# Sorax5/RaytracingEngine

Hardware: AMD Instinct MI355X
Metric: Mrays/sec (primary+shadow) at 1920x1080 (higher is better)
Workload: dtype f64

## Files before the change

### include/rt_capi.h

```cpp
#ifndef RT_CAPI_H
#define RT_CAPI_H

#include <stddef.h>
#include <stdint.h>

#ifdef __cplusplus
extern "C" {
#endif

#define RT_CAPI_VERSION 1

typedef enum rt_status {
    RT_OK = 0,
    RT_ERR_INVALID_ARG = 1,
    RT_ERR_HIP = 2,
    RT_ERR_OOM = 3,
    RT_ERR_UNSUPPORTED = 4,
    RT_ERR_NO_DEVICE = 5,
    RT_ERR_RCCL = 6
} rt_status;

typedef struct rt_material {
    double color[3];
    double shininess;
// ... 197 lines not shown
                            int nframes, const rt_render_opts* opts, int outputs,
                            const struct rt_gbuffer* d_out);
rt_status rt_gbuffer(rt_context* ctx, const rt_scene* scene, const rt_camera* cam,
                     const rt_render_opts* opts, int outputs, const struct rt_gbuffer* h_out);

typedef struct rt_queue rt_queue;
rt_status rt_queue_create(rt_context* ctx, int depth, rt_queue** out);
rt_status rt_queue_destroy(rt_queue* queue);
rt_status rt_queue_submit(rt_queue* queue, const rt_scene* scene, const rt_camera* cam,
                          const rt_render_opts* opts, void* d_hdr64, void* d_hdr32, void* d_ldr,
                          uint64_t* ticket);
rt_status rt_queue_wait(rt_queue* queue, uint64_t ticket);
rt_status rt_queue_synchronize(rt_queue* queue);

rt_status rt_stats_read(rt_context* ctx, rt_stats* out);
rt_status rt_stats_reset(rt_context* ctx);

rt_status rt_trace_rays(rt_context* ctx, const rt_scene* scene, const rt_render_opts* opts,
                        const double* rays, size_t n, double* rgb_out, rt_stats* stats);

rt_status rt_intersect_rays(rt_context* ctx, const rt_scene* scene, const double* rays,
                            size_t n, double* hits_out);

rt_status rt_occluded_rays(rt_context* ctx, const rt_scene* scene, const rt_render_opts* opts,
                           const double* rays, const double* max_dist, size_t n,
                           uint8_t* occluded_out);
rt_status rt_occluded_rays_device(rt_context* ctx, const rt_scene* scene,
                                  const rt_render_opts* opts, const void* d_rays,
                                  const void* d_max_dist, size_t n, void* d_occluded);

rt_status rt_transmittance_rays(rt_context* ctx, const rt_scene* scene, const rt_render_opts* opts,
                                const double* rays, const double* max_dist, size_t n,
                                double* T_out);
rt_status rt_transmittance_rays_device(rt_context* ctx, const rt_scene* scene,
                                       const rt_render_opts* opts, const void* d_rays,
                                       const void* d_max_dist, size_t n, void* d_T);

rt_status rt_light_transmittance(rt_context* ctx, const rt_scene* scene, const rt_render_opts* opts,
                                 const double* points, size_t n, double* T_out);
rt_status rt_light_transmittance_device(rt_context* ctx, const rt_scene* scene,
                                        const rt_render_opts* opts, const void* d_points, size_t n,
                                        void* d_T);

#define RT_DL_RADIANCE 0x1
#define RT_DL_DIFFUSE  0x2
#define RT_DL_SPECULAR 0x4
#define RT_DL_ALL      0x7
struct rt_direct_light_out {
    void* radiance;
    void* diffuse;
    void* specular;
};
rt_status rt_direct_light(rt_context* ctx, const rt_scene* scene, const rt_render_opts* opts,
                          const double* points, const rt_material* materials, size_t n_materials,
                          size_t n, int outputs, const struct rt_direct_light_out* out);
rt_status rt_direct_light_device(rt_context* ctx, const rt_scene* scene,
                                 const rt_render_opts* opts, const void* d_points,
                                 const void* d_materials, size_t n_materials, size_t n,
                                 int outputs, const struct rt_direct_light_out* d_out);

rt_status rt_direct_light_rays(rt_context* ctx, const rt_scene* scene, const rt_render_opts* opts,
                               const double* rays, size_t n, int outputs,
                               const struct rt_direct_light_out* out);
rt_status rt_direct_light_rays_device(rt_context* ctx, const rt_scene* scene,
                                      const rt_render_opts* opts, const void* d_rays, size_t n,
                                      int outputs, const struct rt_direct_light_out* d_out);

#define RT_SC_VALUE    0x01
#define RT_SC_REFRACT  0x02
#define RT_SC_REFLECT  0x04
#define RT_SC_WEIGHTS  0x08
#define RT_SC_FLAGS    0x10
#define RT_SC_ALL      0x1f
struct rt_scatter_out {
    void* value;
    void* refract_rays;
    void* reflect_rays;
    void* weights;
    void* flags;
};
rt_status rt_scatter_rays(rt_context* ctx, const rt_scene* scene, const rt_render_opts* opts,
                          const double* rays, size_t n, int outputs,
                          const struct rt_scatter_out* out);
rt_status rt_scatter_rays_device(rt_context* ctx, const rt_scene* scene,
                                 const rt_render_opts* opts, const void* d_rays, size_t n,
                                 int outputs, const struct rt_scatter_out* d_out);

rt_status rt_camera_rays(rt_context* ctx, const rt_camera* cam, const rt_render_opts* opts,
                         int sample, double* rays_out);
rt_status rt_camera_rays_device(rt_context* ctx, const rt_camera* cam, const rt_render_opts* opts,
                                int sample, void* d_rays);

#define RT_CH_T        0x01
#define RT_CH_PRIM     0x02
#define RT_CH_NORMAL   0x04
#define RT_CH_POINT    0x08
#define RT_CH_MATERIAL 0x10
#define RT_CH_ALL      0x1f
struct rt_closest_out {
    void* t;
    void* prim;
    void* normal;
    void* point;
    void* material;
};
rt_status rt_closest_rays(rt_context* ctx, const rt_scene* scene, const rt_render_opts* opts,
                          const double* rays, size_t n, int outputs,
                          const struct rt_closest_out* out);
rt_status rt_closest_rays_device(rt_context* ctx, const rt_scene* scene,
                                 const rt_render_opts* opts, const void* d_rays, size_t n,
                                 int outputs, const struct rt_closest_out* d_out);

rt_status rt_trace_rays_device(rt_context* ctx, const rt_scene* scene, const rt_render_opts* opts,
                               const void* d_rays, size_t n, void* d_rgb);

rt_status rt_accumulate_samples_device(rt_context* ctx, const rt_scene* scene,
                                       const rt_camera* cam, const rt_render_opts* opts,
                                       int sample_begin, int sample_end, void* d_sum);
rt_status rt_accumulate_samples(rt_context* ctx, const rt_scene* scene, const rt_camera* cam,
                                const rt_render_opts* opts, int sample_begin, int sample_end,
                                double* sum);

rt_status rt_resolve_device(rt_context* ctx, const void* d_sum, size_t n_pixels, int samples,
                            int tonemap, void* d_hdr64, void* d_hdr32, void* d_ldr);
rt_status rt_resolve(rt_context* ctx, const double* sum, size_t n_pixels, int samples, int tonemap,
                     double* hdr64, float* hdr32, uint8_t* ldr);

rt_status rt_tonemap(rt_context* ctx, const double* hdr, size_t n_pixels, int op,
                     uint8_t* ldr_out);

rt_status rt_debug_f64_ops(rt_context* ctx, const double* x, const double* y, size_t n,
                           double* out);

rt_status rt_debug_vec_ops(rt_context* ctx, const double* v, size_t n, double* out);

rt_status rt_debug_assemble_rows(rt_context* ctx, const void* gathered, size_t row_bytes,
                                 uint32_t height, uint32_t block, uint32_t n, uint32_t max_rows,
                                 void* image);

rt_status rt_debug_tile_order(rt_context* ctx, const rt_scene* scene, const rt_camera* cam,
                              uint32_t* order, uint32_t* cost, size_t capacity, uint32_t* tiles,
                              uint32_t* waves, int* state);

rt_status rt_debug_cone_table(rt_context* ctx, uint64_t* with_table, uint64_t* without_table);

rt_status rt_debug_shadow_table(rt_context* ctx, uint64_t* with_table, uint64_t* without_table);

rt_status rt_debug_tile_class(rt_context* ctx, uint64_t* with_words, uint64_t* without_words);

rt_status rt_debug_plane_clear(rt_context* ctx, uint64_t* with_masks, uint64_t* without_masks);

rt_status rt_debug_tile_split(rt_context* ctx, uint64_t* split, uint64_t* single);

#ifdef __cplusplus
}
#endif

#endif
```

### raytracingengine_amd/capi.py

```python
from __future__ import annotations

import ctypes
import os

import numpy as np

from .scene import AREA_LIGHT_DTYPE, SceneData

HERE = os.path.dirname(os.path.abspath(__file__))
LIB_PATH = os.environ.get("RTAMD_LIB", os.path.join(HERE, "librtamd.so"))

(RT_OK, RT_ERR_INVALID_ARG, RT_ERR_HIP, RT_ERR_OOM, RT_ERR_UNSUPPORTED, RT_ERR_NO_DEVICE,
 RT_ERR_RCCL) = range(7)
STATUS_NAMES = {0: "RT_OK", 1: "RT_ERR_INVALID_ARG", 2: "RT_ERR_HIP", 3: "RT_ERR_OOM",
                4: "RT_ERR_UNSUPPORTED", 5: "RT_ERR_NO_DEVICE", 6: "RT_ERR_RCCL"}

TONEMAP_NONE = -1
TONEMAPS = ["simple", "reinhard_simple", "reinhard_extended", "reinhard_extended_luminance",
            "reinhard_jodie", "uncharted2", "aces"]
TONEMAP_ALL = 7
RT_FLAG_COUNT_RAYS = 0x1
RT_FLAG_TIME_KERNEL = 0x2
RT_FLAG_GENERIC_KERNEL = 0x4
RT_FLAG_NO_BVH = 0x8
RT_FLAG_PIPELINE = 0x10
RT_FLAG_NO_TILE_ORDER = 0x20
RT_FLAG_NO_SAMPLE_PARALLEL = 0x40
RT_OUT_HDR64, RT_OUT_HDR32, RT_OUT_LDR = 0x1, 0x2, 0x4
RT_COMM_ID_BYTES = 128
GB_DEPTH = 0x01
GB_DEPTH_NORM = 0x02
GB_NORMAL = 0x04
GB_PRIM = 0x08
GB_ALBEDO = 0x10
GB_ALL = 0x1F
DL_RADIANCE = 0x1
DL_DIFFUSE = 0x2
DL_SPECULAR = 0x4
DL_ALL = 0x7
DL_OUTPUTS = [("radiance", DL_RADIANCE), ("diffuse", DL_DIFFUSE), ("specular", DL_SPECULAR)]
SC_VALUE = 0x01
SC_REFRACT = 0x02
SC_REFLECT = 0x04
SC_WEIGHTS = 0x08
SC_FLAGS = 0x10
SC_ALL = 0x1F
SC_OUTPUTS = [("value", SC_VALUE, np.float64, 3), ("refract_rays", SC_REFRACT, np.float64, 6),
              ("reflect_rays", SC_REFLECT, np.float64, 6), ("weights", SC_WEIGHTS, np.float64, 2),
              ("flags", SC_FLAGS, np.uint8, 0)]
CH_T = 0x01
CH_PRIM = 0x02
CH_NORMAL = 0x04
CH_POINT = 0x08
CH_MATERIAL = 0x10
CH_ALL = 0x1F
CH_OUTPUTS = [("t", CH_T, np.float64, 0), ("prim", CH_PRIM, np.int32, 2),
              ("normal", CH_NORMAL, np.float64, 3), ("point", CH_POINT, np.float64, 3),
              ("material", CH_MATERIAL, np.float64, 7)]
GB_OUTPUTS = [("depth", GB_DEPTH, np.float64, 1), ("depth_norm", GB_DEPTH_NORM, np.float32, 1),
              ("normal", GB_NORMAL, np.float64, 3), ("prim", GB_PRIM, np.int32, 2),
              ("albedo", GB_ALBEDO, np.float32, 3)]

EXPORTED = [
    "rt_last_error", "rt_build_info", "rt_device_count", "rt_render_opts_default", "rt_context_create",
    "rt_context_destroy", "rt_context_set_stream", "rt_context_synchronize", "rt_scene_create",
    "rt_scene_destroy", "rt_scene_set_area_light", "rt_render", "rt_render_device",
    "rt_render_multi", "rt_comm_unique_id", "rt_comm_create", "rt_comm_create_all",
    "rt_comm_create_local", "rt_comm_destroy", "rt_comm_info", "rt_comm_set_root_weight",
    "rt_comm_create_ex", "rt_comm_set_timeout", "rt_render_gather", "rt_render_gather_all",
    "rt_comm_timing", "rt_comm_synchronize", "rt_debug_assemble_rows", "rt_debug_tile_order",
    "rt_stats_read", "rt_stats_reset", "rt_trace_rays", "rt_intersect_rays", "rt_tonemap",
    "rt_debug_f64_ops", "rt_debug_vec_ops", "rt_queue_create", "rt_queue_destroy",
    "rt_queue_submit", "rt_queue_wait", "rt_queue_synchronize", "rt_render_batch",
    "rt_render_gather_batch", "rt_render_gather_all_batch", "rt_gbuffer", "rt_gbuffer_device",
    "rt_debug_cone_table",
    "rt_debug_shadow_table",
    "rt_debug_tile_class",
    "rt_debug_plane_clear",
    "rt_debug_tile_split",
    "rt_occluded_rays", "rt_occluded_rays_device",
    "rt_transmittance_rays", "rt_transmittance_rays_device",
    "rt_light_transmittance", "rt_light_transmittance_device",
    "rt_direct_light", "rt_direct_light_device",
    "rt_direct_light_rays", "rt_direct_light_rays_device",
    "rt_scatter_rays", "rt_scatter_rays_device",
    "rt_camera_rays", "rt_camera_rays_device",
    "rt_closest_rays", "rt_closest_rays_device",
    "rt_trace_rays_device",
    "rt_accumulate_samples", "rt_accumulate_samples_device",
    "rt_resolve", "rt_resolve_device",
]


class RtError(RuntimeError):
    def __init__(self, status: int, msg: str):
        super().__init__(f"{STATUS_NAMES.get(status, status)}: {msg}")
        self.status = status


class SceneDesc(ctypes.Structure):
    _fields_ = [
        ("spheres", ctypes.c_void_p), ("n_spheres", ctypes.c_int32),
        ("planes", ctypes.c_void_p), ("n_planes", ctypes.c_int32),
        ("triangles", ctypes.c_void_p), ("n_triangles", ctypes.c_int32),
        ("lights", ctypes.c_void_p), ("n_lights", ctypes.c_int32),
    ]


class RenderOpts(ctypes.Structure):
    _fields_ = [
        ("max_recursion", ctypes.c_int32), ("tonemap", ctypes.c_int32),
        ("bias", ctypes.c_double), ("seed", ctypes.c_uint64),
        ("row_begin", ctypes.c_uint32), ("row_end", ctypes.c_uint32),
        ("flags", ctypes.c_int32), ("row_block", ctypes.c_uint16), ("row_cycle", ctypes.c_uint16),
    ]


class Stats(ctypes.Structure):
    _fields_ = [
        ("trace_rays", ctypes.c_uint64), ("shadow_rays", ctypes.c_uint64),
        ("kernel_ms", ctypes.c_double), ("launches", ctypes.c_uint64),
    ]


class GBufferPtrs(ctypes.Structure):
    _fields_ = [(name, ctypes.c_void_p) for name, _, _, _ in GB_OUTPUTS]


def gbuffer_layout(outputs: int, width: int, rows: int, frames: int | None = None) -> dict:
    if outputs == 0 or outputs & ~GB_ALL:
        raise ValueError(f"G-buffer outputs {outputs:#x}: no output or an unknown bit")
    lead = () if frames is None else (int(frames),)
    return {name: (lead + (rows, width) + ((k,) if k > 1 else ()), np.dtype(dt))
            for name, bit, dt, k in GB_OUTPUTS if outputs & bit}


class DirectLightPtrs(ctypes.Structure):
    _fields_ = [(name, ctypes.c_void_p) for name, _ in DL_OUTPUTS]


def material_rows(materials, n: int) -> np.ndarray:
    if hasattr(materials, "as_tuple"):
        c, *rest = materials.as_tuple()
        materials = (*c, *rest)
    m = np.ascontiguousarray(materials, np.float64)
    if m.ndim == 1:
        m = m.reshape(1, -1)
    if m.ndim != 2 or m.shape[1] != 7 or m.shape[0] not in (1, n):
        raise ValueError("materials: a Material, seven values, or an [n, 7] array")
    return m


class ScatterPtrs(ctypes.Structure):
    _fields_ = [(name, ctypes.c_void_p) for name, *_ in SC_OUTPUTS]


def _sc_check(outputs: int):
    if outputs == 0 or outputs & ~SC_ALL:
        raise ValueError("outputs: a non-empty combination of SC_* bits")


class ClosestPtrs(ctypes.Structure):
    _fields_ = [(name, ctypes.c_void_p) for name, *_ in CH_OUTPUTS]


def _ch_check(outputs: int):
    if outputs == 0 or outputs & ~CH_ALL:
        raise ValueError("outputs: a non-empty combination of CH_* bits")


def _dl_check(outputs: int):
    if outputs == 0 or outputs & ~DL_ALL:
        raise ValueError("outputs: a non-empty combination of DL_* bits")


class GatherTiming(ctypes.Structure):
    _fields_ = [
        ("render_ms", ctypes.c_double), ("gather_ms", ctypes.c_double),
        ("assemble_ms", ctypes.c_double), ("frames", ctypes.c_uint64),
        ("rows", ctypes.c_uint32), ("max_rows", ctypes.c_uint32),
    ]


_lib = None


def load_library(path: str = LIB_PATH):
    global _lib
    if _lib is not None:
        return _lib
    try:
        import torch
    except ImportError:
        pass
    if not os.path.exists(path):
        raise RuntimeError(
            f"{path} is missing: build it with `python -c 'import __graft_entry__ as g; g.build()'`"
            " (hipcc --offload-arch=gfx950). The renderer has no CPU fallback.")
    L = ctypes.CDLL(path)
    vp, i32 = ctypes.c_void_p, ctypes.c_int
    L.rt_last_error.restype = ctypes.c_char_p
    if hasattr(L, "rt_build_info") or "RTAMD_LIB" not in os.environ:
        L.rt_build_info.restype = ctypes.c_char_p
        L.rt_build_info.argtypes = []
    L.rt_device_count.restype = i32
    L.rt_render_opts_default.argtypes = [vp]
    L.rt_render_opts_default.restype = None
    for name, args in {
        "rt_context_create": [i32, vp],
        "rt_context_destroy": [vp],
        "rt_context_set_stream": [vp, vp],
        "rt_context_synchronize": [vp],
        "rt_scene_create": [vp, vp, vp],
        "rt_scene_destroy": [vp],
        "rt_scene_set_area_light": [vp, vp],
        "rt_render": [vp, vp, vp, vp, vp, vp, vp, vp],
        "rt_render_device": [vp, vp, vp, vp, vp, vp, vp],
        "rt_render_batch": [vp, vp, vp, i32, vp, vp, vp, vp],
        "rt_gbuffer": [vp, vp, vp, vp, i32, vp],
        "rt_gbuffer_device": [vp, vp, vp, i32, vp, i32, vp],
        "rt_render_multi": [vp, vp, i32, vp, vp, vp, vp, vp, vp],
        "rt_stats_read": [vp, vp],
        "rt_stats_reset": [vp],
        "rt_trace_rays": [vp, vp, vp, vp, ctypes.c_size_t, vp, vp],
        "rt_intersect_rays": [vp, vp, vp, ctypes.c_size_t, vp],
        "rt_occluded_rays": [vp, vp, vp, vp, vp, ctypes.c_size_t, vp],
        "rt_occluded_rays_device": [vp, vp, vp, vp, vp, ctypes.c_size_t, vp],
        "rt_transmittance_rays": [vp, vp, vp, vp, vp, ctypes.c_size_t, vp],
        "rt_transmittance_rays_device": [vp, vp, vp, vp, vp, ctypes.c_size_t, vp],
        "rt_light_transmittance": [vp, vp, vp, vp, ctypes.c_size_t, vp],
        "rt_light_transmittance_device": [vp, vp, vp, vp, ctypes.c_size_t, vp],
        "rt_direct_light": [vp, vp, vp, vp, vp, ctypes.c_size_t, ctypes.c_size_t, i32, vp],
        "rt_direct_light_device": [vp, vp, vp, vp, vp, ctypes.c_size_t, ctypes.c_size_t, i32, vp],
        "rt_direct_light_rays": [vp, vp, vp, vp, ctypes.c_size_t, i32, vp],
        "rt_direct_light_rays_device": [vp, vp, vp, vp, ctypes.c_size_t, i32, vp],
        "rt_scatter_rays": [vp, vp, vp, vp, ctypes.c_size_t, i32, vp],
        "rt_scatter_rays_device": [vp, vp, vp, vp, ctypes.c_size_t, i32, vp],
        "rt_camera_rays": [vp, vp, vp, i32, vp],
        "rt_camera_rays_device": [vp, vp, vp, i32, vp],
        "rt_closest_rays": [vp, vp, vp, vp, ctypes.c_size_t, i32, vp],
        "rt_closest_rays_device": [vp, vp, vp, vp, ctypes.c_size_t, i32, vp],
        "rt_trace_rays_device": [vp, vp, vp, vp, ctypes.c_size_t, vp],
        "rt_accumulate_samples": [vp, vp, vp, vp, i32, i32, vp],
        "rt_accumulate_samples_device": [vp, vp, vp, vp, i32, i32, vp],
        "rt_resolve": [vp, vp, ctypes.c_size_t, i32, i32, vp, vp, vp],
        "rt_resolve_device": [vp, vp, ctypes.c_size_t, i32, i32, vp, vp, vp],
        "rt_tonemap": [vp, vp, ctypes.c_size_t, i32, vp],
        "rt_debug_f64_ops": [vp, vp, vp, ctypes.c_size_t, vp],
        "rt_debug_vec_ops": [vp, vp, ctypes.c_size_t, vp],
        "rt_comm_unique_id": [vp],
        "rt_comm_create": [vp, i32, i32, vp, vp],
        "rt_comm_create_ex": [vp, i32, i32, vp, ctypes.c_long, vp],
        "rt_comm_set_timeout": [vp, ctypes.c_long],
        "rt_comm_create_all": [vp, i32, vp],
        "rt_comm_create_local": [vp, i32, vp],
        "rt_comm_destroy": [vp],
        "rt_comm_info": [vp, vp, vp],
        "rt_comm_set_root_weight": [vp, i32],
        "rt_render_gather": [vp, vp, vp, vp, i32, vp, vp, vp],
        "rt_render_gather_all": [vp, vp, i32, vp, vp, i32, vp, vp, vp],
        "rt_render_gather_batch": [vp, vp, vp, i32, vp, i32, vp, vp, vp, vp, vp, vp],
        "rt_render_gather_all_batch": [vp, vp, i32, vp, i32, vp, i32, vp, vp, vp],
        "rt_comm_timing": [vp, vp, i32],
        "rt_comm_synchronize": [vp],
        "rt_queue_create": [vp, i32, vp],
        "rt_queue_destroy": [vp],
        "rt_queue_submit": [vp, vp, vp, vp, vp, vp, vp, vp],
        "rt_queue_wait": [vp, ctypes.c_uint64],
        "rt_queue_synchronize": [vp],
        "rt_debug_tile_order": [vp, vp, vp, vp, vp, ctypes.c_size_t, vp, vp, vp],
        "rt_debug_cone_table": [vp, vp, vp],
        "rt_debug_shadow_table": [vp, vp, vp],
        "rt_debug_tile_class": [vp, vp, vp],
        "rt_debug_plane_clear": [vp, vp, vp],
        "rt_debug_tile_split": [vp, vp, vp],
        "rt_debug_assemble_rows": [vp, vp, ctypes.c_size_t, ctypes.c_uint32, ctypes.c_uint32,
                                   ctypes.c_uint32, ctypes.c_uint32, vp],
    }.items():
        try:
            fn = getattr(L, name)
        except AttributeError:
            if "RTAMD_LIB" in os.environ:
                continue
            raise
        fn.argtypes = args
        fn.restype = i32
    _lib = L
    return L


def build_info() -> dict:
    import json
    info = json.loads(load_library().rt_build_info().decode())
    from . import build
    info["matches_tree"] = info.get("source_sha256") == build.source_digest()
    return info


def _check(status: int):
    if status != RT_OK:
        raise RtError(status, _lib.rt_last_error().decode(errors="replace"))


def rendered_rows(o: RenderOpts, height: int) -> int:
    r1 = min(o.row_end, height) if o.row_end else height
    if r1 <= o.row_begin:
        return 0
    if o.row_cycle <= 1 or o.row_block == 0:
        return r1 - o.row_begin
    stride = o.row_block * o.row_cycle
    return sum(min(o.row_block, r1 - b) for b in range(o.row_begin, r1, stride))


def default_opts(**kw) -> RenderOpts:
    o = RenderOpts()
    load_library().rt_render_opts_default(ctypes.byref(o))
    for k, v in kw.items():
        setattr(o, k, v)
    return o


def device_count() -> int:
    return load_library().rt_device_count()


def progressive_schedule(aa_samples: int) -> list:
    n = max(1, int(aa_samples))
    steps, k = [], 1
    while k < n:
        steps.append(k)
        k *= 2
    return steps + [n]


class Context:

    def __init__(self, device: int = 0):
        L = load_library()
        self._h = ctypes.c_void_p()
        _check(L.rt_context_create(device, ctypes.byref(self._h)))
        self.device = device

    def close(self):
        if self._h:
            _lib.rt_context_destroy(self._h)
            self._h = ctypes.c_void_p()

    def __del__(self):
        try:
            self.close()
        except Exception:
            pass

    def __enter__(self):
        return self

    def __exit__(self, *exc):
        self.close()

    @property
    def handle(self):
        return self._h

    def set_stream(self, stream_ptr: int | None):
        _check(_lib.rt_context_set_stream(self._h, stream_ptr))

    def synchronize(self):
        _check(_lib.rt_context_synchronize(self._h))

    def scene(self, sc: SceneData) -> "DeviceScene":
        return DeviceScene(self, sc)

    def stats(self) -> Stats:
        s = Stats()
        _check(_lib.rt_stats_read(self._h, ctypes.byref(s)))
        return s

    def reset_stats(self):
        _check(_lib.rt_stats_reset(self._h))

    def tonemap(self, hdr: np.ndarray, op: int) -> np.ndarray:
        hdr = np.ascontiguousarray(hdr, np.float64).reshape(-1, 3)
        planes = 7 if op == TONEMAP_ALL else 1
        out = np.empty((planes, hdr.shape[0], 3), np.uint8)
        _check(_lib.rt_tonemap(self._h, hdr.ctypes.data, hdr.shape[0], op, out.ctypes.data))
        return out if planes > 1 else out[0]

    def debug_f64_ops(self, x: np.ndarray, y: np.ndarray) -> np.ndarray:
        x = np.ascontiguousarray(x, np.float64)
        y = np.ascontiguousarray(y, np.float64)
        out = np.empty((x.size, 5), np.float64)
        _check(_lib.rt_debug_f64_ops(self._h, x.ctypes.data, y.ctypes.data, x.size,
                                     out.ctypes.data))
        return out

    def debug_assemble_rows(self, gathered: np.ndarray, height: int, block: int, n: int,
                            max_rows: int) -> np.ndarray:
        g = np.ascontiguousarray(gathered, np.uint8).reshape(n, max_rows, -1)
        out = np.empty((height, g.shape[2]), np.uint8)
        _check(_lib.rt_debug_assemble_rows(self._h, g.ctypes.data, g.shape[2], height, block, n,
                                           max_rows, out.ctypes.data))
        return out

    def debug_cone_table(self) -> tuple[int, int]:
        a, b = ctypes.c_uint64(), ctypes.c_uint64()
        _check(_lib.rt_debug_cone_table(self._h, ctypes.byref(a), ctypes.byref(b)))
        return a.value, b.value

    def debug_shadow_table(self) -> tuple[int, int]:
        a, b = ctypes.c_uint64(), ctypes.c_uint64()
        _check(_lib.rt_debug_shadow_table(self._h, ctypes.byref(a), ctypes.byref(b)))
        return a.value, b.value

    def debug_tile_class(self) -> tuple[int, int]:
        a, b = ctypes.c_uint64(), ctypes.c_uint64()
        _check(_lib.rt_debug_tile_class(self._h, ctypes.byref(a), ctypes.byref(b)))
        return a.value, b.value

    def debug_plane_clear(self) -> tuple[int, int]:
        a, b = ctypes.c_uint64(), ctypes.c_uint64()
        _check(_lib.rt_debug_plane_clear(self._h, ctypes.byref(a), ctypes.byref(b)))
        return a.value, b.value

    def debug_tile_split(self) -> tuple[int, int]:
        a, b = ctypes.c_uint64(), ctypes.c_uint64()
        _check(_lib.rt_debug_tile_split(self._h, ctypes.byref(a), ctypes.byref(b)))
        return a.value, b.value

    def debug_vec_ops(self, v: np.ndarray) -> np.ndarray:
        v = np.ascontiguousarray(v, np.float64).reshape(-1, 3)
        out = np.empty((v.shape[0], 16), np.float64)
        _check(_lib.rt_debug_vec_ops(self._h, v.ctypes.data, v.shape[0], out.ctypes.data))
        return out


class DeviceScene:

    def __init__(self, ctx: Context, sc: SceneData):
        self.ctx = ctx
        self.data = sc
        self._arrays = (sc.sphere_array(), sc.plane_array(), sc.triangle_array(), sc.light_array())
        sp, pl, tr, lt = self._arrays
        desc = SceneDesc(sp.ctypes.data if len(sp) else None, len(sp),
                         pl.ctypes.data if len(pl) else None, len(pl),
                         tr.ctypes.data if len(tr) else None, len(tr),
                         lt.ctypes.data if len(lt) else None, len(lt))
        self._h = ctypes.c_void_p()
        _check(_lib.rt_scene_create(ctx.handle, ctypes.byref(desc), ctypes.byref(self._h)))
        self.camera = sc.camera.to_struct()
        self._area = None
        if sc.area_light is not None:
            self._area = sc.area_light.to_struct()
            _check(_lib.rt_scene_set_area_light(self._h, self._area.ctypes.data))

    def close(self):
        if self._h:
            _lib.rt_scene_destroy(self._h)
            self._h = ctypes.c_void_p()

    def __del__(self):
        try:
            self.close()
        except Exception:
            pass

    def render(self, *, hdr64=True, hdr32=False, tonemap: int = TONEMAP_NONE, opts=None,
               stats=False, **opt_kw):
        cam = self.data.camera
        o = opts if opts is not None else default_opts(tonemap=tonemap, **opt_kw)
        if opts is None:
            o.tonemap = tonemap
        rows = rendered_rows(o, cam.height)
        out = {}
        a64 = np.empty((rows, cam.width, 3), np.float64) if hdr64 else None
        a32 = np.empty((rows, cam.width, 3), np.float32) if hdr32 else None
        ldr = np.empty((rows, cam.width, 3), np.uint8) if tonemap != TONEMAP_NONE else None
        st = Stats()
        _check(_lib.rt_render(self.ctx.handle, self._h, self.camera.ctypes.data, ctypes.byref(o),
                              a64.ctypes.data if a64 is not None else None,
                              a32.ctypes.data if a32 is not None else None,
                              ldr.ctypes.data if ldr is not None else None,
                              ctypes.byref(st) if stats else None))
        if a64 is not None:
            out["hdr64"] = a64
        if a32 is not None:
            out["hdr32"] = a32
        if ldr is not None:
            out["ldr"] = ldr
        if stats:
            out["trace_rays"] = st.trace_rays
            out["shadow_rays"] = st.shadow_rays
        return out

    def render_host(self, h_hdr64: int | None, h_hdr32: int | None, h_ldr: int | None,
                    opts: RenderOpts, stats: bool = False):
        st = Stats()
        _check(_lib.rt_render(self.ctx.handle, self._h, self.camera.ctypes.data, ctypes.byref(opts),
                              h_hdr64, h_hdr32, h_ldr, ctypes.byref(st) if stats else None))
        return st if stats else None

    def trace_rays(self, rays: np.ndarray, stats=False, **opt_kw):
        rays = np.ascontiguousarray(rays, np.float64).reshape(-1, 6)
        out = np.empty((rays.shape[0], 3), np.float64)
        o = default_opts(**opt_kw)
        st = Stats()
        _check(_lib.rt_trace_rays(self.ctx.handle, self._h, ctypes.byref(o), rays.ctypes.data,
                                  rays.shape[0], out.ctypes.data,
                                  ctypes.byref(st) if stats else None))
        return (out, st) if stats else out

    def intersect_rays(self, rays: np.ndarray) -> np.ndarray:
        rays = np.ascontiguousarray(rays, np.float64).reshape(-1, 6)
        out = np.empty((rays.shape[0], 9), np.float64)
        _check(_lib.rt_intersect_rays(self.ctx.handle, self._h, rays.ctypes.data, rays.shape[0],
                                      out.ctypes.data))
        return out

    def occluded(self, rays: np.ndarray, max_dist, no_bvh: bool = False) -> np.ndarray:
        rays = np.ascontiguousarray(rays, np.float64).reshape(-1, 6)
        n = rays.shape[0]
        dist = np.ascontiguousarray(np.broadcast_to(np.asarray(max_dist, np.float64), (n,)))
        out = np.empty(n, np.uint8)
        o = default_opts(flags=RT_FLAG_NO_BVH if no_bvh else 0)
        _check(_lib.rt_occluded_rays(self.ctx.handle, self._h, ctypes.byref(o), rays.ctypes.data,
                                     dist.ctypes.data, n, out.ctypes.data))
        return out.view(np.bool_)

    def occluded_device(self, rays, max_dist, out=None, no_bvh: bool = False):
        import torch
        dev = torch.device(f"cuda:{self.ctx.device}")
        if rays.dtype != torch.float64 or rays.device != dev or not rays.is_contiguous():
            raise ValueError("rays: a contiguous float64 tensor on the context's device")
        n = rays.numel() // 6
        if rays.numel() != 6 * n:
            raise ValueError("rays: n*6 elements")
        if not torch.is_tensor(max_dist):
            max_dist = torch.full((n,), float(max_dist), dtype=torch.float64, device=dev)
            torch.cuda.current_stream(dev).synchronize()
        if (max_dist.dtype != torch.float64 or max_dist.device != dev or max_dist.numel() != n
                or not max_dist.is_contiguous()):
            raise ValueError("max_dist: a scalar or a contiguous float64 [n] tensor on the device")
        if out is None:
            out = torch.empty(n, dtype=torch.uint8, device=dev)
        elif (out.dtype != torch.uint8 or out.device != dev or out.numel() < n
              or not out.is_contiguous()):
            raise ValueError("out: a contiguous uint8 tensor of at least n elements on the device")
        o = default_opts(flags=RT_FLAG_NO_BVH if no_bvh else 0)
        _check(_lib.rt_occluded_rays_device(self.ctx.handle, self._h, ctypes.byref(o),
                                            rays.data_ptr() if n else None,
                                            max_dist.data_ptr() if n else None, n,
                                            out.data_ptr() if n else None))
        return out

    def transmittance(self, rays: np.ndarray, max_dist, bias: float = 1e-3,
                      no_bvh: bool = False) -> np.ndarray:
        rays = np.ascontiguousarray(rays, np.float64).reshape(-1, 6)
        n = rays.shape[0]
        dist = np.ascontiguousarray(np.broadcast_to(np.asarray(max_dist, np.float64), (n,)))
        out = np.empty(n, np.float64)
        o = default_opts(bias=bias, flags=RT_FLAG_NO_BVH if no_bvh else 0)
        _check(_lib.rt_transmittance_rays(self.ctx.handle, self._h, ctypes.byref(o),
                                          rays.ctypes.data, dist.ctypes.data, n, out.ctypes.data))
        return out

    def transmittance_device(self, rays, max_dist, out=None, bias: float = 1e-3,
                             no_bvh: bool = False):
        import torch
        dev = torch.device(f"cuda:{self.ctx.device}")
        if rays.dtype != torch.float64 or rays.device != dev or not rays.is_contiguous():
            raise ValueError("rays: a contiguous float64 tensor on the context's device")
        n = rays.numel() // 6
        if rays.numel() != 6 * n:
            raise ValueError("rays: n*6 elements")
        if not torch.is_tensor(max_dist):
            max_dist = torch.full((n,), float(max_dist), dtype=torch.float64, device=dev)
            torch.cuda.current_stream(dev).synchronize()
        if (max_dist.dtype != torch.float64 or max_dist.device != dev or max_dist.numel() != n
                or not max_dist.is_contiguous()):
            raise ValueError("max_dist: a scalar or a contiguous float64 [n] tensor on the device")
        if out is None:
# ... 631 lines not shown
```

### raytracingengine_amd/csrc/rt_capi.cpp

```cpp
#include "rt_capi.h"

#include <hip/hip_runtime.h>

#include <algorithm>
#include <cmath>
#include <cstdlib>
#include <cstdio>
#include <cstring>
#include <mutex>
#include <new>
#include <string>
#include <utility>
#include <vector>

#include "rt_context.hpp"
#include "rt_internal.hpp"
#include "rt_wavefront.hpp"

#pragma clang fp contract(off)

using namespace rtamd;

namespace rtamd {

// ... 171 lines not shown
                                  static_cast<size_t>(kLtStride) * sc->nl);
    lds = lds_bytes <= ctx->lds_limit;
    return RT_OK;
}

bool uses_wavefront_arena(int path, int flags) {
    if (flags & RT_FLAG_GENERIC_KERNEL) return false;
    const char* wf_chain = std::getenv("RTAMD_WF_CHAIN");
    return path == kPathTree || (path == kPathChain && wf_chain && std::atoi(wf_chain) == 1);
}

rt_status scratch_wait(rt_context* ctx) {
    if (ctx->scratch_used && ctx->scratch_stream != ctx->stream)
        RT_HIP(hipStreamWaitEvent(ctx->stream, ctx->scratch_event, 0));
    return RT_OK;
}

rt_status scratch_done(rt_context* ctx) {
    RT_HIP(hipEventRecord(ctx->scratch_event, ctx->stream));
    ctx->scratch_used = true;
    ctx->scratch_stream = ctx->stream;
    return RT_OK;
}

rt_status fixup_buffers(rt_context* ctx, size_t px, TraceParams& p) {
    if (px >= (size_t(1) << 32)) return fail(RT_ERR_UNSUPPORTED, "fix-up list above 2^32 pixels");
    if (!ctx->fix_ctl.ptr) {
        RT_HIP(ctx->fix_ctl.ensure(2 * sizeof(uint32_t)));
        RT_HIP(hipMemsetAsync(ctx->fix_ctl.ptr, 0, 2 * sizeof(uint32_t), ctx->stream));
    }
    if (ctx->fix_list.bytes < px * sizeof(uint32_t)) {
        if (ctx->scratch_used) RT_HIP(hipEventSynchronize(ctx->scratch_event));
        RT_HIP(ctx->fix_list.ensure(px * sizeof(uint32_t)));
    }
    p.fix_list = static_cast<uint32_t*>(ctx->fix_list.ptr);
    p.fix_ctl = static_cast<uint32_t*>(ctx->fix_ctl.ptr) + ctx->fix_parity;
    p.fix_next = static_cast<uint32_t*>(ctx->fix_ctl.ptr) + (1 - ctx->fix_parity);
    return RT_OK;
}

rt_status check_batch(const rt_camera* cams, int nframes) {
    if (!cams || nframes < 1) return fail(RT_ERR_INVALID_ARG, "frame batch: no cameras");
    for (int f = 0; f < nframes; ++f) {
        rt_status st = validate_camera(cams + f);
        if (st != RT_OK) return st;
        if (cams[f].width != cams[0].width || cams[f].height != cams[0].height ||
            cams[f].aa_samples != cams[0].aa_samples ||
            std::memcmp(&cams[f].focal, &cams[0].focal, sizeof(double)) != 0)
            return fail(RT_ERR_INVALID_ARG, "frame batch: every camera must have the first's "
                                            "width, height, focal and aa_samples");
    }
    return RT_OK;
}

rt_status enqueue_render(rt_context* ctx, const rt_scene* sc, const rt_camera* cam,
                         const rt_render_opts* opts, double* d64, float* d32, uint8_t* dldr) {
    return enqueue_frames(ctx, sc, cam, 1, opts, d64, d32, dldr);
}

rt_status enqueue_frames(rt_context* ctx, const rt_scene* sc, const rt_camera* cams, int nframes,
                         const rt_render_opts* opts, double* d64, float* d32, uint8_t* dldr,
                         uint32_t frame_rows) {
    TraceParams p;
    int path;
    bool lds;
    size_t lds_bytes;
    uint32_t rows;
    rt_status st = nframes == 1 ? RT_OK : check_batch(cams, nframes);
    if (st != RT_OK) return st;
    st = build_params(ctx, sc, cams, opts, p, path, lds, lds_bytes, rows);
    if (st != RT_OK) return st;
    p.out64 = d64;
    p.out32 = d32;
    p.ldr = dldr;
    const int flags = opts ? opts->flags : 0;
    if (!dldr) p.tonemap = RT_TONEMAP_NONE;
    if (dldr && p.tonemap == RT_TONEMAP_NONE) p.ldr = nullptr;
    const bool packet_path = path == kPathDirect && !(flags & RT_FLAG_GENERIC_KERNEL) &&
                             p.ns <= packet_max_spheres() &&
                             packet_lds_bytes(p.ns, p.np, p.nl) <= ctx->lds_limit;
    if (frame_rows && frame_rows < rows)
        return fail(RT_ERR_INVALID_ARG, "frame batch: frame stride below the rendered rows");
    const size_t frame_px = static_cast<size_t>(frame_rows ? frame_rows : rows) * p.width;
    if (nframes > 1 && (!packet_path || nframes > kPkMaxBatch)) {
        const int step = packet_path ? kPkMaxBatch : 1;
        for (int f0 = 0; f0 < nframes; f0 += step) {
            const size_t off = 3 * frame_px * static_cast<size_t>(f0);
            st = enqueue_frames(ctx, sc, cams + f0, std::min(step, nframes - f0), opts,
                                d64 ? d64 + off : nullptr, d32 ? d32 + off : nullptr,
                                dldr ? dldr + off : nullptr, frame_rows);
            if (st != RT_OK) return st;
        }
        return RT_OK;
    }
    bool scratch = (flags & RT_FLAG_COUNT_RAYS) || uses_wavefront_arena(path, flags);

    std::pair<hipEvent_t, hipEvent_t> ev{nullptr, nullptr};
    if (flags & RT_FLAG_TIME_KERNEL) {
        if (ctx->pending.size() >= 1024) {
            st = harvest_events(ctx, false);
            if (st != RT_OK) return st;
        }
        if (!ctx->free_events.empty()) {
            ev = ctx->free_events.back();
            ctx->free_events.pop_back();
        } else {
            RT_HIP(hipEventCreate(&ev.first));
            RT_HIP(hipEventCreate(&ev.second));
        }
        RT_HIP(hipEventRecord(ev.first, ctx->stream));
    }
    const bool packet = packet_path;
    rt_scene::PkImage::TileOrder* rec = nullptr;
    int batch_ring = -1;
    PkSplit pk_split{0u, 0u, 0u};
    if (packet && nframes > 1) {
        p.nframes = static_cast<uint32_t>(nframes);
        p.frame_px = frame_px;
        st = packet_batch_images(ctx, sc, cams, nframes, p, flags, &rec, &batch_ring, &pk_split);
        if (st != RT_OK) return st;
    } else if (packet) {
        st = packet_image(ctx, sc, p, flags, &rec);
        if (st != RT_OK) return st;
    }
    if (packet) {
        for (int f = 0; f < nframes; ++f)
            ++((nframes > 1 ? p.fr_tab[f] : p.cone_tab) ? ctx->cone_tab_frames
                                                         : ctx->cone_notab_frames);
        for (int f = 0; f < nframes; ++f)
            ++((nframes > 1 ? p.fr_stab[f] : p.shadow_tab) ? ctx->shadow_tab_frames
                                                            : ctx->shadow_notab_frames);
        for (int f = 0; f < nframes; ++f)
            ++((nframes > 1 ? p.fr_ctab[f] : p.class_tab) ? ctx->tile_class_frames
                                                          : ctx->tile_noclass_frames);
        for (int f = 0; f < nframes; ++f)
            ++(((nframes > 1 ? p.fr_ctab[f] : p.class_tab) && p.plane_masks)
                   ? ctx->plane_mask_frames
                   : ctx->plane_nomask_frames);
    }
    const bool fixup = packet && packet_uses_fixup(p, false, sc->max_specular > 0.0);
    if (fixup) {
        st = fixup_buffers(ctx, nframes > 1 ? static_cast<size_t>(nframes) * frame_px
                                             : static_cast<size_t>(rows) * p.width, p);
        if (st != RT_OK) return st;
        scratch = true;
    }
    if (scratch) {
        st = scratch_wait(ctx);
        if (st != RT_OK) return st;
    }
    if (!fixup || p.tile_order) pk_split.tiles = 0;
    if (packet && fixup)
        (pk_split.tiles ? ctx->tile_split_frames : ctx->tile_nosplit_frames) += nframes;
    const bool lean_generic = p.nt == 0 && p.al_samples == 0;
    static const bool box_sph = [] {
        const char* e = std::getenv("RTAMD_BOX_SPH");
        return !(e && std::atoi(e) == 0);
    }();
    const bool box = path == kPathChain && p.nt == 0 && p.al_samples == 0 &&
                     (p.ns == 0 ? p.np > 0 : (box_sph && p.ns <= kBoxMaxSpheres)) &&
                     !(flags & RT_FLAG_GENERIC_KERNEL);
    const bool spar = !(flags & RT_FLAG_NO_SAMPLE_PARALLEL);
    auto launch = [&](const TraceParams& q, bool count) {
        if (box)
            return launch_box_chain(q, count, !(flags & RT_FLAG_NO_SAMPLE_PARALLEL), ctx->stream);
        return packet ? launch_packet_direct(q, count, sc->max_specular > 0.0, ctx->stream,
                                             count ? nullptr : &pk_split)
                      : (lean_generic ? lean::launch_trace(q, path, count, lds, lds_bytes, ctx->stream, spar)
                                      : launch_trace(q, path, count, lds, lds_bytes, ctx->stream, spar));
    };
    bool wavefront = false;
    if (uses_wavefront_arena(path, flags)) {
        const size_t n0 = static_cast<size_t>(rows) * p.width *
                          static_cast<size_t>(p.aa > 0 ? p.aa : 0);
        const char* env = std::getenv("RTAMD_WF_MB");
        const size_t budget = (env && std::atoll(env) > 0 ? static_cast<size_t>(std::atoll(env))
                                                          : size_t(4096)) << 20;
        const bool defer = path == kPathTree && wf_defer_selected();
        const size_t root_bytes = wf_arena_bytes(n0, n0, defer);
        if (n0 < (size_t(1) << 30) && root_bytes <= budget) {
            size_t extra = (budget - root_bytes) / (defer ? 116 : 100);
            extra = std::min(extra, std::max<size_t>(n0, 1) * 64);
            extra = std::min(extra, (size_t(1) << 31) - 1 - n0);
            const size_t cap = n0 + extra;
            RT_HIP(ctx->wf.ensure(wf_arena_bytes(n0, cap, defer)));
            RT_HIP(ctx->wf_ctl.ensure(sizeof(WfCtl)));
            const WfArena A = wf_arena_layout(ctx->wf.ptr, n0, cap,
                                              static_cast<WfCtl*>(ctx->wf_ctl.ptr), defer);
            RT_HIP(lean_generic ? lean::launch_wavefront(p, path, A, lds, lds_bytes, ctx->stream)
                                : launch_wavefront(p, path, A, lds, lds_bytes, ctx->stream));
            wavefront = true;
        }
    }
    if (!wavefront) RT_HIP(launch(p, false));
    if (fixup) {
        const hipError_t fe = launch_packet_fixup(p, ctx->stream);
        if (fe != hipSuccess) {
            (void)hipMemsetAsync(ctx->fix_ctl.ptr, 0, 2 * sizeof(uint32_t), ctx->stream);
            return hip_fail(fe, "launch_packet_fixup");
        }
        ctx->fix_parity ^= 1;
    }
    if (rec) RT_HIP(hipEventRecord(rec->recorded, ctx->stream));
    if (flags & RT_FLAG_TIME_KERNEL) {
        RT_HIP(hipEventRecord(ev.second, ctx->stream));
        ctx->pending.push_back(ev);
    }
    if (flags & RT_FLAG_COUNT_RAYS) {
        TraceParams pc = p;
        pc.out64 = nullptr;
        pc.out32 = nullptr;
        pc.ldr = nullptr;
        pc.counters = static_cast<unsigned long long*>(ctx->counters.ptr);
        pc.tile_cost = nullptr;
        RT_HIP(launch(pc, true));
    }
    if (batch_ring >= 0) {
        RT_HIP(hipEventRecord(sc->pk_batch_done[batch_ring], ctx->stream));
        sc->pk_batch_used[batch_ring] = true;
    }
    return scratch ? scratch_done(ctx) : RT_OK;
}

constexpr size_t kGbBytes[5] = {8, 4, 24, 8, 12};

rt_status check_gbuffer_args(int outputs, const rt_gbuffer_out* out) {
    if (outputs == 0) return fail(RT_ERR_INVALID_ARG, "G-buffer: no output requested");
    if (outputs & ~RT_GB_ALL) return fail(RT_ERR_INVALID_ARG, "G-buffer: unknown output bit");
    if (!out) return fail(RT_ERR_INVALID_ARG, "G-buffer: the output record is NULL");
    const void* ptr[5] = {out->depth, out->depth_norm, out->normal, out->prim, out->albedo};
    for (int k = 0; k < 5; ++k)
        if ((outputs & (1 << k)) && !ptr[k])
            return fail(RT_ERR_INVALID_ARG, "G-buffer: a requested output's pointer is NULL");
    return RT_OK;
}

rt_status enqueue_gbuffer(rt_context* ctx, const rt_scene* sc, const rt_camera* cams, int nframes,
                          const rt_render_opts* opts_in, int outputs, const rt_gbuffer_out& out) {
    rt_status st = check_batch(cams, nframes);
    if (st != RT_OK) return st;
    rt_render_opts opts;
    if (opts_in) opts = *opts_in;
    else rt_render_opts_default(&opts);
    opts.max_recursion = 1;
    opts.tonemap = RT_TONEMAP_NONE;
    opts.flags &= RT_FLAG_GENERIC_KERNEL | RT_FLAG_NO_BVH | RT_FLAG_TIME_KERNEL;
    TraceParams p;
    int path;
    bool lds;
    size_t lds_bytes;
    uint32_t rows;
    st = build_params(ctx, sc, cams, &opts, p, path, lds, lds_bytes, rows);
    if (st != RT_OK) return st;
    const bool packet = !(opts.flags & RT_FLAG_GENERIC_KERNEL) &&
                        gbuffer_packet_fits(p, ctx->lds_limit);
    if (packet) p.nl = 0;
    p.frame_px = static_cast<uint64_t>(rows) * p.width;
    GbOut g;

    std::pair<hipEvent_t, hipEvent_t> ev{nullptr, nullptr};
    if (opts.flags & RT_FLAG_TIME_KERNEL) {
        if (ctx->pending.size() >= 1024) {
            st = harvest_events(ctx, false);
            if (st != RT_OK) return st;
        }
        if (!ctx->free_events.empty()) {
            ev = ctx->free_events.back();
            ctx->free_events.pop_back();
        } else {
            RT_HIP(hipEventCreate(&ev.first));
            RT_HIP(hipEventCreate(&ev.second));
        }
        RT_HIP(hipEventRecord(ev.first, ctx->stream));
    }
    for (int f0 = 0; f0 < nframes; f0 += kPkMaxBatch) {
        const int n = std::min(kPkMaxBatch, nframes - f0);
        p.nframes = static_cast<uint32_t>(n);
        for (int f = 0; f < n; ++f) {
            for (int i = 0; i < 3; ++i) p.fr[f].cam[i] = cams[f0 + f].position[i];
            g.planes[f][0] = cams[f0 + f].near_plane;
            g.planes[f][1] = cams[f0 + f].far_plane;
        }
        const size_t off = static_cast<size_t>(f0) * p.frame_px;
        auto at = [&](void* base, int bit, size_t elems) -> char* {
            return (outputs & bit) ? static_cast<char*>(base) + off * elems : nullptr;
        };
        g.depth = reinterpret_cast<double*>(at(out.depth, RT_GB_DEPTH, kGbBytes[0]));
        g.depth_norm = reinterpret_cast<float*>(at(out.depth_norm, RT_GB_DEPTH_NORM, kGbBytes[1]));
        g.normal = reinterpret_cast<double*>(at(out.normal, RT_GB_NORMAL, kGbBytes[2]));
        g.prim = reinterpret_cast<int32_t*>(at(out.prim, RT_GB_PRIM, kGbBytes[3]));
        g.albedo = reinterpret_cast<float*>(at(out.albedo, RT_GB_ALBEDO, kGbBytes[4]));
        RT_HIP(launch_gbuffer(p, g, packet, 0, ctx->stream));
    }
    if (opts.flags & RT_FLAG_TIME_KERNEL) {
        RT_HIP(hipEventRecord(ev.second, ctx->stream));
        ctx->pending.push_back(ev);
    }
    return RT_OK;
}

}

extern "C" {

const char* rt_last_error(void) { return g_last_error.c_str(); }

// ... 1154 lines not shown
    return RT_OK;
}

rt_status rt_resolve_device(rt_context* ctx, const void* d_sum, size_t n, int samples, int tonemap,
                            void* d_hdr64, void* d_hdr32, void* d_ldr) {
    rt_status st = check_resolve_args(ctx, d_sum, n, samples, tonemap, d_hdr64, d_hdr32, d_ldr,
                                      "rt_resolve_device");
    if (st != RT_OK) return st;
    if (n == 0) return RT_OK;
    DeviceGuard g(ctx->device);
    RT_HIP(launch_resolve(static_cast<const double*>(d_sum), n, samples, tonemap,
                          static_cast<double*>(d_hdr64), static_cast<float*>(d_hdr32),
                          static_cast<uint8_t*>(d_ldr), ctx->stream));
    return RT_OK;
}

rt_status rt_resolve(rt_context* ctx, const double* sum, size_t n, int samples, int tonemap,
                     double* hdr64, float* hdr32, uint8_t* ldr) {
    rt_status st = check_resolve_args(ctx, sum, n, samples, tonemap, hdr64, hdr32, ldr, "rt_resolve");
    if (st != RT_OK) return st;
    if (n == 0) return RT_OK;
    DeviceGuard g(ctx->device);
    const size_t planes = tonemap == RT_TONEMAP_COUNT ? RT_TONEMAP_COUNT : 1;
    RT_HIP(ctx->tm_in.ensure(n * 3 * sizeof(double)));
    if (hdr64) RT_HIP(ctx->out64.ensure(n * 3 * sizeof(double)));
    if (hdr32) RT_HIP(ctx->out32.ensure(n * 3 * sizeof(float)));
    if (ldr) RT_HIP(ctx->tm_out.ensure(planes * n * 3));
    RT_HIP(hipMemcpyAsync(ctx->tm_in.ptr, sum, n * 3 * sizeof(double), hipMemcpyHostToDevice,
                          ctx->stream));
    RT_HIP(launch_resolve(static_cast<const double*>(ctx->tm_in.ptr), n, samples, tonemap,
                          hdr64 ? static_cast<double*>(ctx->out64.ptr) : nullptr,
                          hdr32 ? static_cast<float*>(ctx->out32.ptr) : nullptr,
                          ldr ? static_cast<uint8_t*>(ctx->tm_out.ptr) : nullptr, ctx->stream));
    if (hdr64)
        RT_HIP(hipMemcpyAsync(hdr64, ctx->out64.ptr, n * 3 * sizeof(double), hipMemcpyDeviceToHost,
                              ctx->stream));
    if (hdr32)
        RT_HIP(hipMemcpyAsync(hdr32, ctx->out32.ptr, n * 3 * sizeof(float), hipMemcpyDeviceToHost,
                              ctx->stream));
    if (ldr)
        RT_HIP(hipMemcpyAsync(ldr, ctx->tm_out.ptr, planes * n * 3, hipMemcpyDeviceToHost,
                              ctx->stream));
    RT_HIP(hipStreamSynchronize(ctx->stream));
    return RT_OK;
}

rt_status rt_tonemap(rt_context* ctx, const double* hdr, size_t n, int op, uint8_t* out) {
    if (!ctx || (!hdr && n) || (!out && n))
        return fail(RT_ERR_INVALID_ARG, "NULL argument to rt_tonemap");
    if (op < 0 || op > RT_TONEMAP_COUNT) return fail(RT_ERR_INVALID_ARG, "tonemap op out of range");
    if (n == 0) return RT_OK;
    DeviceGuard g(ctx->device);
    const size_t planes = op == RT_TONEMAP_COUNT ? RT_TONEMAP_COUNT : 1;
    RT_HIP(ctx->tm_in.ensure(n * 3 * sizeof(double)));
    RT_HIP(ctx->tm_out.ensure(planes * n * 3));
    RT_HIP(hipMemcpyAsync(ctx->tm_in.ptr, hdr, n * 3 * sizeof(double), hipMemcpyHostToDevice,
                          ctx->stream));
    RT_HIP(launch_tonemap(static_cast<const double*>(ctx->tm_in.ptr), n, op,
                          static_cast<uint8_t*>(ctx->tm_out.ptr), ctx->stream));
    RT_HIP(hipMemcpyAsync(out, ctx->tm_out.ptr, planes * n * 3, hipMemcpyDeviceToHost,
                          ctx->stream));
    RT_HIP(hipStreamSynchronize(ctx->stream));
    return RT_OK;
}

rt_status rt_debug_f64_ops(rt_context* ctx, const double* x, const double* y, size_t n,
                           double* out) {
    if (!ctx || !x || !y || !out) return fail(RT_ERR_INVALID_ARG, "NULL argument");
    DeviceGuard g(ctx->device);
    RT_HIP(ctx->dbg.ensure(n * 7 * sizeof(double)));
    double* dx = static_cast<double*>(ctx->dbg.ptr);
    double* dy = dx + n;
    double* dout = dy + n;
    RT_HIP(hipMemcpyAsync(dx, x, n * sizeof(double), hipMemcpyHostToDevice, ctx->stream));
    RT_HIP(hipMemcpyAsync(dy, y, n * sizeof(double), hipMemcpyHostToDevice, ctx->stream));
    RT_HIP(launch_debug_f64(dx, dy, n, dout, ctx->stream));
    RT_HIP(hipMemcpyAsync(out, dout, 5 * n * sizeof(double), hipMemcpyDeviceToHost, ctx->stream));
    RT_HIP(hipStreamSynchronize(ctx->stream));
    return RT_OK;
}

rt_status rt_debug_tile_order(rt_context* ctx, const rt_scene* sc, const rt_camera* cam,
                              uint32_t* order, uint32_t* cost, size_t capacity, uint32_t* tiles,
                              uint32_t* waves, int* state) {
    if (!ctx || !sc || !cam || !tiles || !waves || !state)
        return fail(RT_ERR_INVALID_ARG, "NULL argument to rt_debug_tile_order");
    *tiles = *waves = 0;
    *state = 0;
    DeviceGuard g(ctx->device);
    RT_HIP(hipDeviceSynchronize());
    for (const auto& im : sc->pk_images) {
        if (std::memcmp(im.cam, cam->position, sizeof im.cam) != 0) continue;
        if (im.last_ord < 0) return RT_OK;
        const auto& o = im.ords[static_cast<size_t>(im.last_ord)];
        *state = o.state;
        if (o.state == 0) return RT_OK;
        *tiles = o.key[0] * o.key[1];
        *waves = o.key[2];
        if (order && o.state == 2) {
            if (capacity < *tiles) return fail(RT_ERR_INVALID_ARG, "order capacity too small");
            RT_HIP(hipMemcpy(order, o.order.ptr, sizeof(uint32_t) * *tiles, hipMemcpyDeviceToHost));
        }
        if (cost) {
            if (capacity < size_t(*tiles) * *waves)
                return fail(RT_ERR_INVALID_ARG, "cost capacity too small");
            RT_HIP(hipMemcpy(cost, o.cost.ptr, sizeof(uint32_t) * *tiles * *waves,
                             hipMemcpyDeviceToHost));
        }
        return RT_OK;
    }
    return RT_OK;
}

rt_status rt_debug_cone_table(rt_context* ctx, uint64_t* with_table, uint64_t* without_table) {
    if (!ctx || !with_table || !without_table)
        return fail(RT_ERR_INVALID_ARG, "NULL argument to rt_debug_cone_table");
    *with_table = ctx->cone_tab_frames;
    *without_table = ctx->cone_notab_frames;
    return RT_OK;
}

rt_status rt_debug_shadow_table(rt_context* ctx, uint64_t* with_table, uint64_t* without_table) {
    if (!ctx || !with_table || !without_table)
        return fail(RT_ERR_INVALID_ARG, "NULL argument to rt_debug_shadow_table");
    *with_table = ctx->shadow_tab_frames;
    *without_table = ctx->shadow_notab_frames;
    return RT_OK;
}

rt_status rt_debug_tile_class(rt_context* ctx, uint64_t* with_words, uint64_t* without_words) {
    if (!ctx || !with_words || !without_words)
        return fail(RT_ERR_INVALID_ARG, "NULL argument to rt_debug_tile_class");
    *with_words = ctx->tile_class_frames;
    *without_words = ctx->tile_noclass_frames;
    return RT_OK;
}

rt_status rt_debug_plane_clear(rt_context* ctx, uint64_t* with_masks, uint64_t* without_masks) {
    if (!ctx || !with_masks || !without_masks)
        return fail(RT_ERR_INVALID_ARG, "NULL argument to rt_debug_plane_clear");
    *with_masks = ctx->plane_mask_frames;
    *without_masks = ctx->plane_nomask_frames;
    return RT_OK;
}

rt_status rt_debug_tile_split(rt_context* ctx, uint64_t* split, uint64_t* single) {
    if (!ctx || !split || !single)
        return fail(RT_ERR_INVALID_ARG, "NULL argument to rt_debug_tile_split");
    *split = ctx->tile_split_frames;
    *single = ctx->tile_nosplit_frames;
    return RT_OK;
}

rt_status rt_debug_vec_ops(rt_context* ctx, const double* v, size_t n, double* out) {
    if (!ctx || !v || !out) return fail(RT_ERR_INVALID_ARG, "NULL argument");
    DeviceGuard g(ctx->device);
    RT_HIP(ctx->dbg.ensure(n * 19 * sizeof(double)));
    double* dv = static_cast<double*>(ctx->dbg.ptr);
    double* dout = dv + 3 * n;
    RT_HIP(hipMemcpyAsync(dv, v, 3 * n * sizeof(double), hipMemcpyHostToDevice, ctx->stream));
    RT_HIP(launch_debug_vec(dv, n, dout, ctx->stream));
    RT_HIP(hipMemcpyAsync(out, dout, 16 * n * sizeof(double), hipMemcpyDeviceToHost, ctx->stream));
    RT_HIP(hipStreamSynchronize(ctx->stream));
    return RT_OK;
}

}
```

### raytracingengine_amd/csrc/rt_context.hpp

```cpp
#pragma once

#include <hip/hip_runtime.h>

#include <array>
#include <string>
#include <utility>
#include <vector>

#include "rt_capi.h"
#include "rt_internal.hpp"

namespace rtamd {

rt_status fail(rt_status st, const std::string& msg);
rt_status hip_fail(hipError_t e, const char* what);

#define RT_HIP(call)                                    \
    do {                                                \
        hipError_t e_ = (call);                         \
        if (e_ != hipSuccess) return rtamd::hip_fail(e_, #call); \
    } while (0)

struct DeviceBuffer {
    void* ptr = nullptr;
    size_t bytes = 0;
    hipError_t ensure(size_t need) {
        if (need <= bytes) return hipSuccess;
        if (ptr) (void)hipFree(ptr);
        ptr = nullptr;
        bytes = 0;
        hipError_t e = hipMalloc(&ptr, need);
        if (e == hipSuccess) bytes = need;
        return e;
    }
    void release() {
        if (ptr) (void)hipFree(ptr);
        ptr = nullptr;
        bytes = 0;
    }
};

struct DeviceGuard {
    int prev = -1;
    explicit DeviceGuard(int dev) {
        if (hipGetDevice(&prev) != hipSuccess) prev = -1;
        (void)hipSetDevice(dev);
    }
    ~DeviceGuard() {
        if (prev >= 0) (void)hipSetDevice(prev);
    }
};

}

struct rt_comm;

struct rt_context {
    int device = 0;
    hipStream_t stream = nullptr;
    hipStream_t own_stream = nullptr;
    size_t lds_limit = 0;
    rtamd::DeviceBuffer out64, out32, ldr, tm_in, tm_out, dbg, rays;
    rtamd::DeviceBuffer counters;
    rtamd::DeviceBuffer wf, wf_ctl;
    hipEvent_t scratch_event = nullptr;
    bool scratch_used = false;
    hipStream_t scratch_stream = nullptr;
    rtamd::DeviceBuffer fix_list, fix_ctl;
    int fix_parity = 0;
    std::vector<std::pair<hipEvent_t, hipEvent_t>> pending;
    std::vector<std::pair<hipEvent_t, hipEvent_t>> free_events;
    double timed_ms = 0.0;
    uint64_t launches = 0;
    uint64_t cone_tab_frames = 0, cone_notab_frames = 0;
    uint64_t shadow_tab_frames = 0, shadow_notab_frames = 0;
    uint64_t tile_class_frames = 0, tile_noclass_frames = 0;
    uint64_t plane_mask_frames = 0, plane_nomask_frames = 0;
    uint64_t tile_split_frames = 0, tile_nosplit_frames = 0;
    std::vector<rt_context*> group_ctxs;
    std::vector<rt_comm*> group_comms;
    std::vector<rt_context*> group_roots;
};

struct rt_scene {
    rt_context* ctx = nullptr;
    rtamd::DeviceBuffer buf;
    int32_t ns = 0, np = 0, nt = 0, nl = 0;
    size_t off_sph = 0, off_sph_mat = 0, off_pl = 0, off_pl_mat = 0, off_tri = 0, off_tri_mat = 0,
           off_lt = 0;
    bool any_transparent = false;
    double max_specular = 0.0;
    bool has_area = false;
    rt_area_light area{};
    size_t off_bvh = 0, off_bvh_tri = 0;
    int32_t bvh_nodes = 0;
    size_t off_sperm = 0, off_sbnd = 0;
    size_t off_box = 0;
    int32_t box_n[4] = {0, 0, 0, 0};
    struct PkImage {
        double cam[3];
        rtamd::DeviceBuffer buf;
        hipEvent_t ready = nullptr;
        hipStream_t stream = nullptr;
        bool done = false;
        struct TileOrder {
            uint32_t key[8] = {};
            int state = 0;
            rtamd::DeviceBuffer cost, keys, order;
            hipEvent_t recorded = nullptr, built = nullptr;
            uint32_t* verdict = nullptr;
        };
        std::vector<TileOrder> ords;
        int last_ord = -1;
        struct ConeTab {
            static constexpr size_t kKeyWords = 20;
            uint32_t key[kKeyWords] = {};
            rtamd::DeviceBuffer buf;
            hipEvent_t ready = nullptr;
            hipStream_t stream = nullptr;
            bool done = false;
            unsigned long long* counts = nullptr;
        };
        std::vector<ConeTab> tabs;
    };
    mutable std::vector<PkImage> pk_images;
    mutable std::vector<std::array<double, 3>> pk_seen;
    mutable rtamd::DeviceBuffer pk_pub;
    static constexpr int kPkBatchRing = 4;
    mutable rtamd::DeviceBuffer pk_batch;
    mutable hipEvent_t pk_batch_done[kPkBatchRing] = {nullptr, nullptr, nullptr, nullptr};
    mutable bool pk_batch_used[kPkBatchRing] = {false, false, false, false};
    mutable int pk_batch_next = 0;
    mutable rtamd::DeviceBuffer pk_batch_tab[kPkBatchRing];
};

namespace rtamd {

uint32_t rendered_rows(const rt_render_opts& o, uint32_t height);
rt_status validate_camera(const rt_camera* cam);
rt_status enqueue_render(rt_context* ctx, const rt_scene* sc, const rt_camera* cam,
                         const rt_render_opts* opts, double* d64, float* d32, uint8_t* dldr);
rt_status enqueue_frames(rt_context* ctx, const rt_scene* sc, const rt_camera* cams, int nframes,
                         const rt_render_opts* opts, double* d64, float* d32, uint8_t* dldr,
                         uint32_t frame_rows = 0);
rt_status check_batch(const rt_camera* cams, int nframes);
rt_status packet_image(rt_context* ctx, const rt_scene* sc, TraceParams& p, int flags,
                       rt_scene::PkImage::TileOrder** rec);
rt_status packet_batch_images(rt_context* ctx, const rt_scene* sc, const rt_camera* cams,
                              int nframes, TraceParams& p, int flags,
                              rt_scene::PkImage::TileOrder** rec, int* batch_ring,
                              PkSplit* split);
bool uses_wavefront_arena(int path, int flags);
rt_status scratch_wait(rt_context* ctx);
rt_status scratch_done(rt_context* ctx);
rt_status harvest_events(rt_context* ctx, bool all);
void release_group(rt_context* ctx);
void leave_groups(rt_context* ctx);

}
```

### raytracingengine_amd/csrc/rt_internal.hpp

```cpp
#pragma once

#include <hip/hip_runtime.h>
#include <stddef.h>
#include <stdint.h>

#include <vector>

namespace rtamd {

constexpr int kSphStride = 4;
constexpr int kPlStride = 8;
constexpr int kTriStride = 12;
constexpr int kLtStride = 8;
constexpr int kMatStride = 8;
constexpr int kBoxRec = 16;
constexpr int kBoxMaxSpheres = 64;

constexpr int kBvhNodeStride = 8;
constexpr int kBvhMinTris = 32;
constexpr int kBvhStack = 64;
constexpr int kMaxDepth = 16;
constexpr int kTileW = 8;
constexpr int kTileH = 32;

enum PathKind : int {
    kPathDirect = 0,
    kPathChain = 1,
    kPathTree = 2
};

constexpr int kPkMaxBatch = 32;
struct PkFrame {
    double cam[3];
    const double* img;
    unsigned long long* pub;
    uint32_t epoch;
    uint32_t _pad;
};

struct TraceParams {
    const double* sph;
    const double* sph_mat;
    const double* pl;
    const double* pl_mat;
    const double* tri;
    const double* tri_mat;
    const double* lt;
    int32_t ns, np, nt, nl;
    double al_corner[3];
    double al_u[3];
    double al_v[3];
    double al_E[3];
    int32_t al_samples;
    int32_t al_k;
    double cam_pos[3];
    double focal;
    uint32_t width, height;
    int32_t aa;
    int32_t max_rec;
    double bias;
    uint64_t seed;
    uint32_t row0, rows;
    uint32_t row_block, row_stride;
    double* out64;
    float* out32;
    uint8_t* ldr;
    int32_t tonemap;
    int32_t _pad;
    unsigned long long* counters;
    const uint8_t* redo;
    const double* bvh;
    const int32_t* bvh_tri;
    const double* pk_image;
    unsigned long long* pk_pub;
    uint32_t pk_epoch;
    uint32_t pk_pub_first;
    const int32_t* sph_perm;
    const double* sph_bnd;
    const uint32_t* redo_any;
    const uint32_t* tile_order;
    uint32_t* tile_cost;
    const double* box;
    int32_t box_n[4];
    uint32_t* fix_list;
    uint32_t* fix_ctl;
    uint32_t* fix_next;
    uint32_t nframes;
    uint32_t plane_masks;
    uint64_t frame_px;
    PkFrame fr[kPkMaxBatch];
    double half_w, half_h, cam_dz, cam_dz2;
    double fr_dz[kPkMaxBatch][2];
    const unsigned long long* cone_tab;
    const unsigned long long* fr_tab[kPkMaxBatch];
    const unsigned long long* shadow_tab;
    const unsigned long long* fr_stab[kPkMaxBatch];
    const unsigned long long* class_tab;
    const unsigned long long* fr_ctab[kPkMaxBatch];
};
struct PkSplit {
    uint32_t tiles;
    uint32_t uni_n, gen_n;
};
static_assert(sizeof(TraceParams) + 12 * kPkMaxBatch + 32 <= 4096, "kernel arguments above 4 KiB");

struct CameraConsts {
    double half_w, half_h, dz, dz2;
};
inline CameraConsts camera_consts(uint32_t width, uint32_t height, double cam_z, double focal) {
    CameraConsts c;
    c.half_w = static_cast<double>(width) / 2.0;
    c.half_h = static_cast<double>(height) / 2.0;
    c.dz = (cam_z + focal) - cam_z;
    c.dz2 = c.dz * c.dz;
    return c;
}

constexpr int kSphChunkMin = 65;
void build_sphere_chunks(const double* sph, int ns, std::vector<int32_t>& perm,
                         std::vector<double>& bounds);

void build_triangle_bvh(const double* tri, int nt, std::vector<double>& nodes,
                        std::vector<int32_t>& order);

__host__ __device__ inline size_t scene_doubles(const TraceParams& p) {
    return static_cast<size_t>(kSphStride) * p.ns + static_cast<size_t>(kPlStride) * p.np +
           static_cast<size_t>(kLtStride) * p.nl;
}

constexpr int kAaParallelMax = 128;
hipError_t launch_trace(const TraceParams& p, int path, bool count, bool lds, size_t lds_bytes,
                        hipStream_t stream, bool sample_parallel = false);
namespace lean {
hipError_t launch_trace(const TraceParams& p, int path, bool count, bool lds, size_t lds_bytes,
                        hipStream_t stream, bool sample_parallel = false);
}
hipError_t launch_box_chain(const TraceParams& p, bool count, bool sample_parallel,
                            hipStream_t stream);
hipError_t launch_packet_direct(const TraceParams& p, bool count, bool any_specular,
                                hipStream_t stream, const PkSplit* split = nullptr);
size_t packet_lds_bytes(int ns, int np, int nl);
hipError_t launch_packet_image(const TraceParams& p, double* img, hipStream_t stream);
bool packet_uses_fixup(const TraceParams& p, bool count, bool any_specular);
hipError_t launch_packet_fixup(const TraceParams& p, hipStream_t stream);
struct PkImageJobs {
    double* dst[kPkMaxBatch];
    int32_t frame[kPkMaxBatch];
    int32_t n;
};
hipError_t launch_packet_image_batch(const TraceParams& p, const PkImageJobs& jobs,
                                     hipStream_t stream);
struct PkConeJobs {
    unsigned long long* dst[kPkMaxBatch];
    int32_t frame[kPkMaxBatch];
    int32_t n;
    int32_t shadow_nl;
    int32_t class_words;
    int32_t lists;
};
struct PkListCounts {
    unsigned long long* host[kPkMaxBatch];
};
hipError_t launch_packet_cone_tables(const TraceParams& p, const PkConeJobs& jobs,
                                     hipStream_t stream, const PkListCounts* counts = nullptr);
bool packet_split_wanted(const TraceParams& p);
bool packet_reads_cone_table(const TraceParams& p, bool any_specular);
int packet_shadow_table_lights(const TraceParams& p);
void packet_grid(const TraceParams& p, uint32_t& gx, uint32_t& gy, uint32_t& waves);
hipError_t launch_packet_order(const uint32_t* cost, uint32_t gx, uint32_t gy, uint32_t waves,
                               uint32_t* keys, uint32_t* order, uint32_t* verdict,
                               hipStream_t stream);
int packet_max_spheres();
struct GbOut {
    double* depth;
    float* depth_norm;
    double* normal;
    int32_t* prim;
    float* albedo;
    double planes[kPkMaxBatch][2];
};
bool gbuffer_packet_fits(const TraceParams& p, size_t lds_limit);
hipError_t launch_gbuffer(const TraceParams& p, const GbOut& g, bool packet, int tile_w,
                          hipStream_t stream);
hipError_t launch_trace_rays(const TraceParams& p, int path, bool count, const double* rays,
                             size_t n, double* out, hipStream_t stream);
hipError_t launch_intersect_rays(const TraceParams& p, const double* rays, size_t n, double* out,
                                 hipStream_t stream);
hipError_t launch_occluded_rays(const TraceParams& p, const double* rays, const double* max_dist,
                                size_t n, uint8_t* out, hipStream_t stream);
hipError_t launch_transmittance_rays(const TraceParams& p, bool opaque, const double* rays,
                                     const double* max_dist, size_t n, double* out,
                                     hipStream_t stream);
hipError_t launch_light_transmittance(const TraceParams& p, bool opaque, const double* points,
                                      size_t n, double* out, hipStream_t stream);
struct DlOut {
    double* radiance;
    double* diffuse;
    double* specular;
};
struct DlMaterial {
    double v[8];
};
hipError_t launch_direct_light_points(const TraceParams& p, bool opaque, const double* points,
                                      const double* materials, const DlMaterial& shared, size_t n,
                                      const DlOut& out, hipStream_t stream);
hipError_t launch_direct_light_rays(const TraceParams& p, bool opaque, const double* rays, size_t n,
                                    const DlOut& out, hipStream_t stream);
struct ScOut {
    double* value;
    double* refract_rays;
    double* reflect_rays;
    double* weights;
    uint8_t* flags;
};
hipError_t launch_scatter_rays(const TraceParams& p, bool opaque, const double* rays, size_t n,
                               const ScOut& out, hipStream_t stream);
hipError_t launch_camera_rays(const TraceParams& p, int sample, double* out, hipStream_t stream);
struct ChOut {
    double* t;
    int32_t* prim;
    double* normal;
    double* point;
    double* material;
};
hipError_t launch_closest_rays(const TraceParams& p, const double* rays, size_t n, const ChOut& out,
                               hipStream_t stream);
hipError_t launch_accumulate_samples(const TraceParams& p, int path, int s0, int s1, double* sum,
                                     hipStream_t stream);
hipError_t launch_resolve(const double* sum, size_t n, int samples, int op, double* out64,
                          float* out32, uint8_t* ldr, hipStream_t stream);
hipError_t launch_tonemap(const double* hdr, size_t n, int op, uint8_t* out, hipStream_t stream);
hipError_t launch_debug_f64(const double* x, const double* y, size_t n, double* out,
                            hipStream_t stream);
hipError_t launch_debug_vec(const double* v, size_t n, double* out, hipStream_t stream);

}
```

### raytracingengine_amd/csrc/rt_packet.hip

```cpp
#include "rt_cone_table.hpp"
#include "rt_packet_kernel.hpp"
#include "rt_shadow_table.hpp"

#pragma clang fp contract(off)

namespace rtamd {

#ifdef RT_PACKET_PROBE
template __global__ void packet_direct_kernel<RT_PACKET_PROBE>(TraceParams);
#else
size_t packet_lds_bytes(int ns, int np, int nl) { return pk_image_bytes(ns, np, nl); }

__global__ __launch_bounds__(256) void packet_image_kernel(TraceParams P, double* img) {
    pk_build_image(P, P.cam_pos, img, static_cast<int>(threadIdx.x), 256);
}

hipError_t launch_packet_image(const TraceParams& p, double* img, hipStream_t stream) {
    hipLaunchKernelGGL(packet_image_kernel, dim3(1), dim3(256), 0, stream, p, img);
    return hipGetLastError();
}

__global__ __launch_bounds__(256) void packet_image_batch_kernel(TraceParams P, PkImageJobs J) {
    const int f = J.frame[blockIdx.x];
    pk_build_image(P, P.fr[f].cam, J.dst[blockIdx.x], static_cast<int>(threadIdx.x), 256);
}

hipError_t launch_packet_image_batch(const TraceParams& p, const PkImageJobs& jobs,
                                     hipStream_t stream) {
    if (jobs.n <= 0) return hipSuccess;
    if (jobs.n > kPkMaxBatch) return hipErrorInvalidValue;
    for (int j = 0; j < jobs.n; ++j)
        if (!jobs.dst[j] || jobs.frame[j] < 0 || jobs.frame[j] >= static_cast<int>(p.nframes))
            return hipErrorInvalidValue;
    hipLaunchKernelGGL(packet_image_batch_kernel, dim3(static_cast<unsigned>(jobs.n)),
                       dim3(256), 0, stream, p, jobs);
    return hipGetLastError();
}

constexpr int kConeThreads = 256;
__global__ __launch_bounds__(kConeThreads, 5) void packet_cone_table_kernel(TraceParams P,
                                                                         PkConeJobs J, uint32_t gx,
                                                                         uint32_t gy,
                                                                         uint32_t waves) {
    __shared__ float s_terms[64 * 8];
    __shared__ double s_ctr[64 * 3];
    const int f = J.frame[blockIdx.y];
    const double* camp = f < 0 ? P.cam_pos : P.fr[f].cam;
    const double* img = f < 0 ? P.pk_image : P.fr[f].img;
    const double dz = f < 0 ? P.cam_dz : P.fr_dz[f][0];
    const int ns = P.ns < 64 ? P.ns : 64;
    for (int i = threadIdx.x; i < 8 * ns; i += kConeThreads)
        s_terms[i] = reinterpret_cast<const float*>(img + kPkSph * (i >> 3) + 4)[i & 7];
    if (J.shadow_nl > 0)
        for (int i = threadIdx.x; i < 3 * ns; i += kConeThreads)
            s_ctr[i] = img[kPkSph * (i / 3) + i % 3];
    __syncthreads();
    const uint32_t pos = blockIdx.x * kConeThreads + threadIdx.x;
    if (pos >= gx * gy * waves) return;
    const uint32_t t = J.lists ? tile_list_tile(pos, gx * gy * waves) : pos;
    const uint32_t wave = t % waves, wg = t / waves, tbx = wg % gx, tby = wg / gx;
    const uint32_t x0 = tbx * (kPkW * kWgWavesX) + (wave % kWgWavesX) * kPkW;
    const uint32_t yl0 = tby * (kPkH * (waves / kWgWavesX)) + (wave / kWgWavesX) * kPkH;
    const ConeRowPlan rp{P.row0, P.rows, P.row_block, P.row_stride};
    const ConeRect q = cone_tile_rect(x0, yl0, P.width, rp);
    const ConeBound B = cone_tile_bound(q, P.half_w, P.half_h, camp[0], camp[1], dz);
    const uint64_t cone = cone_tile_mask(B, s_terms, 8, ns);
    J.dst[blockIdx.y][t] = cone;
    if (J.shadow_nl <= 0) return;
    unsigned long long* sw = J.dst[blockIdx.y] + static_cast<size_t>(gx) * gy * waves +
                             static_cast<size_t>(t) * J.shadow_nl;
    ShadowBound<2> SB;
    SB.n = 0;
    SB.ok = false;
    if (cone == 0)
        SB = shadow_tile_bound<2>(q, P.half_w, P.half_h, camp, dz, img + kPkSph * ns, P.np, P.bias);
    unsigned long long any = 0, keep = 0;
    for (int l = 0; l < J.shadow_nl; ++l) {
        sw[l] = shadow_tile_word(SB, P.lt + kLtStride * l, P.bias, s_ctr, 3, s_terms + 7, 8, ns);
        any |= sw[l];
        const unsigned k = J.class_words == 2
                               ? shadow_plane_keep<2>(SB, P.lt + kLtStride * l, img + kPkSph * ns,
                                                      P.np, camp, P.bias)
                               : kPlaneKeepAll;
        keep |= static_cast<unsigned long long>(k) << (8 + 8 * l);
    }
    if (J.class_words == 0) return;
    const double* pln = img + kPkSph * ns + kPlStride * P.np + kLtStride * P.nl;
    const unsigned long long cw = tile_class_word(cone, SB, &any, 1, pln, P.np) | keep;
    J.dst[blockIdx.y][static_cast<size_t>(gx) * gy * waves * (1 + J.shadow_nl) + t] = cw;
    if (!J.lists) return;
    const size_t tiles = static_cast<size_t>(gx) * gy * waves;
    unsigned long long* hdr = J.dst[blockIdx.y] + tiles * (2 + J.shadow_nl);
    unsigned long long* uni = hdr + 1;
    uint32_t* gen = reinterpret_cast<uint32_t*>(hdr + 1 + tiles);
    const uint32_t lane = threadIdx.x & 63u;
    const bool is_uni = tile_list_uniform(cw);
    const uint64_t bu = __ballot(is_uni), bg = __ballot(!is_uni);
    const bool lead = (lane & (waves - 1u)) == 0 && tile_list_wg_listed(bg, lane, waves);
    const uint64_t bl = __ballot(lead);
    uint32_t base_u = 0, base_g = 0;
    if (lane == 0) {
        if (bu) base_u = atomicAdd(reinterpret_cast<uint32_t*>(hdr),
                                   static_cast<uint32_t>(__builtin_popcountll(bu)));
        if (bl) base_g = atomicAdd(reinterpret_cast<uint32_t*>(hdr) + 1,
                                   static_cast<uint32_t>(__builtin_popcountll(bl)));
    }
    base_u = __shfl(base_u, 0, 64);
    base_g = __shfl(base_g, 0, 64);
    const uint64_t below = (1ull << lane) - 1ull;
    if (is_uni) uni[base_u + __builtin_popcountll(bu & below)] = tile_list_entry(cw, x0, yl0);
    if (lead) gen[base_g + __builtin_popcountll(bl & below)] = wg;
}

__global__ __launch_bounds__(64) void packet_list_zero_kernel(PkConeJobs J, size_t hdr) {
    if (static_cast<int>(threadIdx.x) < J.n) J.dst[threadIdx.x][hdr] = 0ull;
}
__global__ __launch_bounds__(64) void packet_list_counts_kernel(PkConeJobs J, PkListCounts C,
                                                                size_t hdr) {
    if (static_cast<int>(threadIdx.x) >= J.n || !C.host[threadIdx.x]) return;
    const unsigned long long v = J.dst[threadIdx.x][hdr];
    __hip_atomic_store(C.host[threadIdx.x],
                       (((v >> 32) + 1ull) << 32) | ((v & 0xffffffffull) + 1ull), __ATOMIC_RELAXED,
                       __HIP_MEMORY_SCOPE_SYSTEM);
}

hipError_t launch_packet_cone_tables(const TraceParams& p, const PkConeJobs& jobs,
                                     hipStream_t stream, const PkListCounts* counts) {
    if (jobs.n <= 0) return hipSuccess;
    if (jobs.n > kPkMaxBatch || p.ns > 64 || p.width == 0 || p.rows == 0)
        return hipErrorInvalidValue;
    if (jobs.shadow_nl != 0 && jobs.shadow_nl != packet_shadow_table_lights(p))
        return hipErrorInvalidValue;
    if (jobs.class_words != 0 && jobs.shadow_nl <= 0) return hipErrorInvalidValue;
    if (jobs.class_words < 0 || jobs.class_words > 2) return hipErrorInvalidValue;
    if (jobs.lists != 0 && jobs.class_words == 0) return hipErrorInvalidValue;
    for (int j = 0; j < jobs.n; ++j) {
        const int f = jobs.frame[j];
        if (!jobs.dst[j] || f < -1 || f >= static_cast<int>(p.nframes) ||
            !(f < 0 ? p.pk_image : p.fr[f].img))
            return hipErrorInvalidValue;
    }
    uint32_t gx, gy, waves;
    packet_grid(p, gx, gy, waves);
    const uint32_t tiles = gx * gy * waves;
    const size_t hdr = static_cast<size_t>(tiles) * (2 + jobs.shadow_nl);
    if (jobs.lists) {
        if (gx * kWgWavesX > kListMaxCoord || gy * (waves / kWgWavesX) > kListMaxCoord)
            return hipErrorInvalidValue;
        hipLaunchKernelGGL(packet_list_zero_kernel, dim3(1), dim3(64), 0, stream, jobs, hdr);
    }
    hipLaunchKernelGGL(packet_cone_table_kernel,
                       dim3((tiles + kConeThreads - 1) / kConeThreads,
                            static_cast<unsigned>(jobs.n)),
                       dim3(kConeThreads), 0, stream, p, jobs, gx, gy, waves);
    if (jobs.lists && counts)
        hipLaunchKernelGGL(packet_list_counts_kernel, dim3(1), dim3(64), 0, stream, jobs, *counts,
                           hdr);
    return hipGetLastError();
}

constexpr int kFixThreads = 256;
constexpr int kFixBlocks = 256;
template <bool LDS>
__global__ __launch_bounds__(kFixThreads) void packet_fixup_kernel(TraceParams P) {
    extern __shared__ double smem[];
    const uint32_t n = *P.fix_ctl;
    if (blockIdx.x == 0 && threadIdx.x == 0) *P.fix_next = 0u;
    if (blockIdx.x * kFixThreads >= n) return;
    SceneView S = stage_scene<LDS>(P, smem, threadIdx.x, kFixThreads);
    S.nt = 0;
    S.al = 0;
    S.spec = false;
    S.tri = S.tri_mat = S.bvh = nullptr;
    S.bvh_tri = nullptr;
    Counts cnt{0u, 0u};
    const uint32_t fpx = P.nframes ? static_cast<uint32_t>(P.frame_px) : 0u;
    for (uint32_t i = blockIdx.x * kFixThreads + threadIdx.x; i < n; i += gridDim.x * kFixThreads) {
        const uint32_t o = P.fix_list[i];
        const uint32_t z = fpx ? o / fpx : 0u;
        const uint32_t pl = o - z * fpx;
        const uint32_t yl = pl / P.width;
        const uint32_t x = pl - yl * P.width;
        const double* cp = P.nframes ? P.fr[z].cam : P.cam_pos;
        const d3 cam = mk(cp[0], cp[1], cp[2]);
        const uint32_t y = image_row(P, yl);
        const uint64_t pix = static_cast<uint64_t>(y) * P.width + x;
        const d3 d = camera_dir(P, cam, x, y, pix, 0);
        d3 acc = mk(0.0, 0.0, 0.0);
        acc = acc + trace_direct<false>(S, P, cam, d, pix, 0u, cnt);
        store_pixel(P, static_cast<size_t>(o), acc);
    }
}

hipError_t launch_packet_fixup(const TraceParams& p, hipStream_t stream) {
    if (!p.fix_list || !p.fix_ctl || !p.fix_next) return hipErrorInvalidValue;
    if (p.nt != 0 || p.al_samples != 0) return hipErrorInvalidValue;
    const size_t lds = sizeof(double) * scene_doubles(p);
    if (lds <= 32 * 1024)
        hipLaunchKernelGGL(packet_fixup_kernel<true>, dim3(kFixBlocks), dim3(kFixThreads), lds,
                           stream, p);
    else
        hipLaunchKernelGGL(packet_fixup_kernel<false>, dim3(kFixBlocks), dim3(kFixThreads), 0,
                           stream, p);
    return hipGetLastError();
}

int packet_max_spheres() { return 16 * 64; }

void packet_grid(const TraceParams& p, uint32_t& gx, uint32_t& gy, uint32_t& waves) {
    const size_t lds = pk_image_bytes(p.ns, p.np, p.nl);
    const uint32_t wgy = pk_wgy(lds);
    gx = (p.width + kPkW * kWgWavesX - 1) / (kPkW * kWgWavesX);
    gy = (p.rows + kPkH * wgy - 1) / (kPkH * wgy);
    waves = kWgWavesX * wgy;
}

constexpr int kOrderBins = 16;
__global__ __launch_bounds__(1024) void packet_order_kernel(const uint32_t* cost, uint32_t gx,
                                                            uint32_t gy, uint32_t waves,
                                                            uint32_t* keys, uint32_t* order,
                                                            uint32_t* verdict) {
    __shared__ uint32_t s_max, s_cnt[kOrderBins];
    const uint32_t tid = threadIdx.x, tiles = gx * gy;
    if (tid == 0) s_max = 0;
    if (tid < kOrderBins) s_cnt[tid] = 0;
    __syncthreads();
    uint32_t m = 0;
    for (uint32_t i = tid; i < tiles; i += blockDim.x) {
        uint32_t c = 0;
        for (uint32_t w = 0; w < waves; ++w) c = max(c, cost[i * waves + w]);
        keys[i] = c;
        m = max(m, c);
    }
    atomicMax(&s_max, m);
    __syncthreads();
    const uint64_t top = static_cast<uint64_t>(s_max) + 1;
    for (uint32_t i = tid; i < tiles; i += blockDim.x) {
        const uint64_t bin = static_cast<uint64_t>(keys[i]) * kOrderBins / top;
        const uint32_t key = kOrderBins - 1 - static_cast<uint32_t>(bin);
        keys[i] = key;
        atomicAdd(&s_cnt[key], 1u);
    }
    __syncthreads();
    if (tid >= 64) return;
    uint32_t acc = 0;
    int median_bin = 0;
    for (int b = kOrderBins - 1; b >= 0; --b) {
        acc += s_cnt[b];
        if (2 * acc >= tiles) {
            median_bin = kOrderBins - 1 - b;
            break;
        }
    }
    const bool narrow = median_bin >= kOrderBins / 4;
    if (tid == 0 && verdict) __hip_atomic_store(verdict, narrow ? 1u : 2u, __ATOMIC_RELAXED,
                                                __HIP_MEMORY_SCOPE_SYSTEM);
    uint32_t cur = 0;
    for (int b = 0; b < kOrderBins; ++b)
        if (static_cast<int>(tid) > b) cur += s_cnt[b];
    if (narrow) {
        for (uint32_t lin = tid; lin < tiles; lin += 64) order[lin] = (gy - 1 - lin / gx) * gx + lin % gx;
        return;
    }
    const uint64_t below = (1ull << tid) - 1ull;
    for (uint32_t c0 = 0; c0 < tiles; c0 += 64) {
        const uint32_t lin = c0 + tid;
        const bool ok = lin < tiles;
        uint32_t tile = 0, key = kOrderBins;
        if (ok) {
            tile = (gy - 1 - lin / gx) * gx + lin % gx;
            key = keys[tile];
        }
        for (int b = 0; b < kOrderBins; ++b) {
            const uint64_t mk_ = __ballot(key == static_cast<uint32_t>(b));
            if (!mk_) continue;
            const uint32_t base = __builtin_amdgcn_readlane(cur, b);
            if (key == static_cast<uint32_t>(b))
                order[base + __builtin_popcountll(mk_ & below)] = tile;
            if (static_cast<int>(tid) == b) cur += __builtin_popcountll(mk_);
        }
    }
}

hipError_t launch_packet_order(const uint32_t* cost, uint32_t gx, uint32_t gy, uint32_t waves,
                               uint32_t* keys, uint32_t* order, uint32_t* verdict,
                               hipStream_t stream) {
    hipLaunchKernelGGL(packet_order_kernel, dim3(1), dim3(1024), 0, stream, cost, gx, gy, waves,
                       keys, order, verdict);
    return hipGetLastError();
}

template <int MAXC>
static void launch_packet_maxc(const TraceParams& p, bool count, size_t lds, int feat,
                               hipStream_t stream) {
    if (feat == kFeatFix) launch_packet_variant<1, kFeatFix>(p, count, lds, stream);
    else if (feat == 0) launch_packet_variant<MAXC, 0>(p, count, lds, stream);
    else if (feat == kFeatPlanes) launch_packet_variant<MAXC, kFeatPlanes>(p, count, lds, stream);
    else if (feat == kFeatTris) launch_packet_variant<MAXC, kFeatTris>(p, count, lds, stream);
    else launch_packet_variant<MAXC, kFeatAll>(p, count, lds, stream);
}

static int packet_features(const TraceParams& p, bool any_specular) {
    int feat = 0;
    if (any_specular) feat |= kFeatSpec;
    if (p.al_samples > 0) feat |= kFeatArea;
    if (p.nt > 0) feat |= kFeatTris;
    if (p.ldr && p.tonemap == 4) feat |= kFeatJodie;
    if (p.np >= 3 && feat == 0) feat = kFeatPlanes;
    return feat;
}

bool packet_reads_cone_table(const TraceParams& p, bool any_specular) {
    return p.aa == 1 && !p.tile_cost && p.ns >= 1 && p.ns <= 64 && p.max_rec > 0 &&
           packet_features(p, any_specular) == 0;
}

int packet_shadow_table_lights(const TraceParams& p) {
    return p.np <= 2 ? shadow_table_lights(p.ns, p.np, p.nl, p.al_samples > 0) : 0;
}

constexpr uint64_t kPkFixMinPixels = 32ull << 20;
bool packet_uses_fixup(const TraceParams& p, bool count, bool any_specular) {
    const char* e = std::getenv("RTAMD_PK_FIX");
    const int mode = e ? std::atoi(e) : -1;
    if (mode == 0) return false;
    const bool eligible = !count && p.aa == 1 && !p.tile_cost && p.nframes >= 1 &&
                          (p.ns + 63) / 64 <= 1 && packet_features(p, any_specular) == 0;
    const uint64_t px = static_cast<uint64_t>(p.nframes) * p.rows * p.width;
    return eligible && (mode == 1 || px >= kPkFixMinPixels);
}

#ifndef RT_PACKET_UNI_THREADS
#define RT_PACKET_UNI_THREADS 256
#endif
#ifndef RT_PACKET_UNI_WAVES
#define RT_PACKET_UNI_WAVES 8
#endif
constexpr int kUniThreads = RT_PACKET_UNI_THREADS;
__global__ __launch_bounds__(kUniThreads, RT_PACKET_UNI_WAVES) void packet_uniform_kernel(TraceParams P, uint32_t tiles) {
    constexpr int FEAT = kFeatFix;
    const PkFrame& F = P.fr[blockIdx.z];
    const pk_culp hdr = (pk_culp)P.fr_ctab[blockIdx.z] + tiles;
    const uint32_t i = blockIdx.x * (kUniThreads / 64) +
                       __builtin_amdgcn_readfirstlane(static_cast<uint32_t>(threadIdx.x) >> 6);
    if (i >= static_cast<uint32_t>(hdr[0])) return;
    const unsigned long long e = hdr[1 + i];
    const unsigned long long cls = e & kListWordMask;
    const uint32_t col = static_cast<uint32_t>(e >> kListColShift) & kListCoordMask;
    const uint32_t row = static_cast<uint32_t>(e >> kListRowShift) & kListCoordMask;
    const d3 cam = mk(F.cam[0], F.cam[1], F.cam[2]);
    const double cam_dz = P.fr_dz[blockIdx.z][0], cam_dz2 = P.fr_dz[blockIdx.z][1];
    const uint64_t frame_off = static_cast<uint64_t>(blockIdx.z) * P.frame_px;
    const uint32_t lane = __builtin_amdgcn_mbcnt_hi(~0u, __builtin_amdgcn_mbcnt_lo(~0u, 0u));
    const uint32_t x = col * kPkW + (lane % kPkW), yl = row * kPkH + (lane / kPkW);
    const uint32_t xc = x < P.width ? x : P.width - 1;
    const uint32_t y = image_row(P, yl < P.rows ? yl : P.rows - 1);
    const double sx = static_cast<double>(xc) - P.half_w;
    const double sy = P.half_h - static_cast<double>(y);
    const d3 dv = mk(sx - cam.x, sy - cam.y, cam_dz);
    const d3 d = unit_sq(dv, dv.x * dv.x + dv.y * dv.y + cam_dz2);
    bool fix = false;
    PacketScene S;
    S.lt = nullptr;
    const d3 col3 = pk_uniform_tile<1, FEAT>(S, P, F.img, cls, cam, d, P.ns, P.np, P.nl, P.bias, fix);
    const d3 acc = mk(0.0, 0.0, 0.0) + col3;
    constexpr int samples = 1;
    const uint32_t lane_e = lane, x_e = x, yl_e = yl;
#include "rt_packet_epilogue.hpp"
}

bool packet_split_wanted(const TraceParams& p) {
    const char* e = std::getenv("RTAMD_PK_TILE_SPLIT");
    if (e && std::atoi(e) == 0) return false;
    uint32_t gx, gy, waves;
    packet_grid(p, gx, gy, waves);
    return !p.tile_order && waves == kWgWavesX && gx * kWgWavesX <= kListMaxCoord &&
           gy <= kListMaxCoord;
}

static void launch_packet_split(const TraceParams& p, const PkSplit& s, size_t lds,
                                hipStream_t stream) {
    const dim3 block(64 * kWgWavesX);
    const dim3 ggrid(s.gen_n, 1u, p.nframes);
    const dim3 ugrid((s.uni_n + kUniThreads / 64 - 1) / (kUniThreads / 64), 1u, p.nframes);
#ifdef RT_PACKET_SPLIT_GENERAL_FIRST
    if (s.gen_n)
        hipLaunchKernelGGL((packet_direct_kernel<1, kFeatFix | kFeatSplit, false, false, 1>),
                           ggrid, block, lds, stream, p);
#endif
    if (s.uni_n)
        hipLaunchKernelGGL(packet_uniform_kernel, ugrid, dim3(kUniThreads), 0, stream, p,
                           s.tiles);
#ifndef RT_PACKET_SPLIT_GENERAL_FIRST
    if (s.gen_n)
        hipLaunchKernelGGL((packet_direct_kernel<1, kFeatFix | kFeatSplit, false, false, 1>),
                           ggrid, block, lds, stream, p);
#endif
}

hipError_t launch_packet_direct(const TraceParams& p, bool count, bool any_specular,
                                hipStream_t stream, const PkSplit* split) {
    const size_t lds = packet_lds_bytes(p.ns, p.np, p.nl);
    const int chunks = (p.ns + 63) / 64;
    int feat = packet_features(p, any_specular);
    if (packet_uses_fixup(p, count, any_specular)) {
        if (!p.fix_list || !p.fix_ctl || !p.fix_next) return hipErrorInvalidValue;
        feat = kFeatFix;
        if (split && split->tiles) {
            launch_packet_split(p, *split, lds, stream);
            return hipGetLastError();
        }
    }
    if (feat == kFeatArea) return launch_packet_area(p, count, lds, chunks, stream);
    if (chunks <= 1) launch_packet_maxc<1>(p, count, lds, feat, stream);
    else if (chunks <= 4) launch_packet_maxc<4>(p, count, lds, feat, stream);
    else launch_packet_maxc<16>(p, count, lds, feat, stream);
    return hipGetLastError();
}
#endif

}
```

### raytracingengine_amd/csrc/rt_packet_host.cpp

```cpp
#include <hip/hip_runtime.h>

#include <algorithm>
#include <array>
#include <atomic>
#include <cstdlib>
#include <cstring>

#include "rt_context.hpp"
#include "rt_internal.hpp"
#include "rt_shadow_table.hpp"

#pragma clang fp contract(off)

namespace rtamd {
namespace {

constexpr size_t kMaxPkImages = 16;
constexpr size_t kMaxPkSeen = 16;
constexpr size_t kMaxTileOrders = 8;
constexpr size_t kPkPubSlots = 32;
constexpr size_t kPkPubMaxWords = 1024;
std::atomic<uint32_t> g_pk_epoch{0};
rt_status packet_publish_slot(rt_context* ctx, const rt_scene* sc, TraceParams& p) {
    const size_t words = packet_lds_bytes(p.ns, p.np, p.nl) / 4;
    static const bool off = [] {
        const char* e = std::getenv("RTAMD_PK_PUB");
        return e && std::atoi(e) == 0;
    }();
    if (off || words > kPkPubMaxWords) return RT_OK;
    const size_t slot = kPkPubMaxWords * sizeof(unsigned long long);
    if (!sc->pk_pub.ptr) {
        RT_HIP(sc->pk_pub.ensure(kPkPubSlots * slot));
        RT_HIP(hipMemsetAsync(sc->pk_pub.ptr, 0, kPkPubSlots * slot, ctx->stream));
        RT_HIP(hipStreamSynchronize(ctx->stream));
    }
    uint32_t ep = ++g_pk_epoch;
    if (ep == 0) ep = ++g_pk_epoch;
    p.pk_epoch = ep;
    static const long first_env = [] {
        const char* e = std::getenv("RTAMD_PK_PUB_FIRST");
        return e ? std::atol(e) : -1L;
    }();
    int cus = 0;
    RT_HIP(hipDeviceGetAttribute(&cus, hipDeviceAttributeMultiprocessorCount, ctx->device));
    p.pk_pub_first = first_env >= 0 ? static_cast<uint32_t>(first_env)
                                    : static_cast<uint32_t>(cus > 0 ? cus : 256) * 10u;
    p.pk_pub = reinterpret_cast<unsigned long long*>(static_cast<char*>(sc->pk_pub.ptr) +
                                                     (ep % kPkPubSlots) * slot);
    return RT_OK;
}
rt_status tile_order(rt_context* ctx, rt_scene::PkImage& im, TraceParams& p, int flags,
                     rt_scene::PkImage::TileOrder** rec, bool existing_only = false) {
    *rec = nullptr;
    if (flags & RT_FLAG_NO_TILE_ORDER) return RT_OK;
    uint32_t gx, gy, waves;
    packet_grid(p, gx, gy, waves);
    const uint32_t key[8] = {gx, gy, waves, p.width, p.height, p.rows, p.row0,
                             (p.row_block << 16) ^ p.row_stride};
    const uint32_t tiles = gx * gy;
    size_t idx = 0;
    while (idx < im.ords.size() && std::memcmp(im.ords[idx].key, key, sizeof key) != 0) ++idx;
    if (existing_only && (idx == im.ords.size() || im.ords[idx].state != 2)) return RT_OK;
    if (idx == im.ords.size()) {
        if (im.ords.size() >= kMaxTileOrders) return RT_OK;
        if (im.ords.capacity() < kMaxTileOrders) im.ords.reserve(kMaxTileOrders);
        im.ords.emplace_back();
        auto& o = im.ords.back();
        im.last_ord = static_cast<int>(idx);
        hipError_t e = o.cost.ensure(sizeof(uint32_t) * tiles * waves);
        if (e == hipSuccess) e = hipEventCreateWithFlags(&o.recorded, hipEventDisableTiming);
        if (e != hipSuccess) {
            o.cost.release();
            im.ords.pop_back();
            im.last_ord = -1;
            return hip_fail(e, "tile order");
        }
        std::memcpy(o.key, key, sizeof key);
        o.state = 1;
        p.tile_cost = static_cast<uint32_t*>(o.cost.ptr);
        *rec = &o;
        return RT_OK;
    }
    auto& o = im.ords[idx];
    im.last_ord = static_cast<int>(idx);
    if (o.state == 1) {
        RT_HIP(o.keys.ensure(sizeof(uint32_t) * tiles));
        RT_HIP(o.order.ensure(sizeof(uint32_t) * tiles));
        if (!o.built) RT_HIP(hipEventCreateWithFlags(&o.built, hipEventDisableTiming));
        if (!o.verdict) RT_HIP(hipHostMalloc(reinterpret_cast<void**>(&o.verdict), sizeof(uint32_t)));
        __atomic_store_n(o.verdict, 0u, __ATOMIC_RELAXED);
        RT_HIP(hipStreamWaitEvent(ctx->stream, o.recorded, 0));
        RT_HIP(launch_packet_order(static_cast<const uint32_t*>(o.cost.ptr), gx, gy, waves,
                                   static_cast<uint32_t*>(o.keys.ptr),
                                   static_cast<uint32_t*>(o.order.ptr), o.verdict, ctx->stream));
        RT_HIP(hipEventRecord(o.built, ctx->stream));
        o.state = 2;
    } else {
        if (__atomic_load_n(o.verdict, __ATOMIC_RELAXED) == 1u) return RT_OK;
        RT_HIP(hipStreamWaitEvent(ctx->stream, o.built, 0));
    }
    p.tile_order = static_cast<const uint32_t*>(o.order.ptr);
    return RT_OK;
}

rt_status scene_tile_order(rt_context* ctx, const rt_scene* sc, TraceParams& p, int flags,
                           rt_scene::PkImage::TileOrder** rec) {
    for (auto& im : sc->pk_images) {
        const rt_status st = tile_order(ctx, im, p, flags, rec, true);
        if (st != RT_OK || p.tile_order) return st;
    }
    return RT_OK;
}

rt_status packet_image_cached(rt_context* ctx, const rt_scene* sc, const double* cam,
                              rt_scene::PkImage** out) {
    *out = nullptr;
    for (auto& im : sc->pk_images) {
        if (std::memcmp(im.cam, cam, sizeof im.cam) != 0) continue;
        if (!im.done && im.stream != ctx->stream) {
            const hipError_t q = hipEventQuery(im.ready);
            if (q == hipSuccess) im.done = true;
            else if (q == hipErrorNotReady) RT_HIP(hipStreamWaitEvent(ctx->stream, im.ready, 0));
            else return hip_fail(q, "hipEventQuery");
        }
        *out = &im;
        return RT_OK;
    }
    return RT_OK;
}

bool packet_second_sighting(const rt_scene* sc, const double* cam) {
    auto& seen = sc->pk_seen;
    auto it = std::find_if(seen.begin(), seen.end(), [&](const std::array<double, 3>& c) {
        return std::memcmp(c.data(), cam, 3 * sizeof(double)) == 0;
    });
    if (it == seen.end()) {
        if (seen.size() >= kMaxPkSeen) seen.erase(seen.begin());
        seen.push_back({cam[0], cam[1], cam[2]});
        return false;
    }
    if (sc->pk_images.size() >= kMaxPkImages) return false;
    seen.erase(it);
    return true;
}

rt_status packet_image_entry(rt_context* ctx, const rt_scene* sc, const double* cam,
                             const TraceParams& p, rt_scene::PkImage** out) {
    *out = nullptr;
    if (sc->pk_images.capacity() < kMaxPkImages) sc->pk_images.reserve(kMaxPkImages);
    sc->pk_images.emplace_back();
    rt_scene::PkImage& im = sc->pk_images.back();
    std::memcpy(im.cam, cam, sizeof im.cam);
    im.stream = ctx->stream;
    hipError_t e = im.buf.ensure(packet_lds_bytes(p.ns, p.np, p.nl));
    if (e == hipSuccess) e = hipEventCreateWithFlags(&im.ready, hipEventDisableTiming);
    if (e != hipSuccess) {
        im.buf.release();
        if (im.ready) (void)hipEventDestroy(im.ready);
        sc->pk_images.pop_back();
        return hip_fail(e, "packet image entry");
    }
    *out = &im;
    return RT_OK;
}

constexpr size_t kMaxConeTabs = 8;
constexpr size_t kConeRingBytes = size_t(16) << 20;

struct TabsWanted {
    bool cone, shadow;
    int shadow_nl;
    bool cls;
    bool clear;
    bool lists;
    int cls_kind() const { return cls ? (clear ? 2 : 1) : 0; }
    bool any() const { return cone || shadow; }
};
TabsWanted tables_wanted(const rt_scene* sc, const TraceParams& p) {
    TabsWanted w{false, false, 0, false, false, false};
    if (!packet_reads_cone_table(p, sc->max_specular > 0.0)) return w;
    const char* e = std::getenv("RTAMD_PK_CONE_TAB");
    w.cone = !(e && std::atoi(e) == 0);
    e = std::getenv("RTAMD_PK_SHADOW_TAB");
    w.shadow = packet_shadow_table_lights(p) > 0 && !(e && std::atoi(e) == 0);
    w.shadow_nl = w.shadow ? packet_shadow_table_lights(p) : 0;
    e = std::getenv("RTAMD_PK_TILE_CLASS");
    w.cls = w.cone && w.shadow && !(e && std::atoi(e) == 0);
    e = std::getenv("RTAMD_PK_PLANE_CLEAR");
    w.clear = w.cls && !(e && std::atoi(e) == 0);
    w.lists = w.cls && p.nframes >= 1 && packet_uses_fixup(p, false, sc->max_specular > 0.0) &&
              packet_split_wanted(p);
    return w;
}

constexpr size_t kConeKeyWords = rt_scene::PkImage::ConeTab::kKeyWords;
size_t cone_table_key(const TraceParams& p, double dz, int shadow_nl, int cls, bool lists,
                      uint32_t (&key)[kConeKeyWords], size_t* tiles = nullptr) {
    uint32_t gx, gy, waves;
    packet_grid(p, gx, gy, waves);
    const uint32_t k[9] = {gx, gy, waves, p.width, p.height, p.rows, p.row0, p.row_block,
                           p.row_stride};
    const double c[3] = {dz, p.half_w, p.half_h};
    std::memset(key, 0, sizeof key);
    std::memcpy(key, k, sizeof k);
    std::memcpy(key + 9, c, sizeof c);
    static_assert(sizeof k + sizeof c + 2 * sizeof(uint32_t) + sizeof(double) <=
                      sizeof(uint32_t) * kConeKeyWords, "cone table key");
    if (shadow_nl > 0) {
        key[15] = static_cast<uint32_t>(shadow_nl);
        std::memcpy(key + 16, &p.bias, sizeof p.bias);
        key[18] = (cls == 2 ? 3u : (cls ? 1u : 0u)) | (cls && lists ? 4u : 0u);
    }
    const size_t n = static_cast<size_t>(gx) * gy * waves;
    if (tiles) *tiles = n;
    return sizeof(unsigned long long) *
           (n * (1 + static_cast<size_t>(shadow_nl > 0 ? shadow_nl + (cls ? 1 : 0) : 0)) +
            (shadow_nl > 0 && cls && lists ? tile_list_words(n, static_cast<size_t>(gx) * gy) : 0));
}

rt_status cone_table_entry(rt_context* ctx, rt_scene::PkImage& im, const TraceParams& p,
                           double dz, int shadow_nl, int cls, bool lists,
                           rt_scene::PkImage::ConeTab** tab, bool* fresh) {
    *tab = nullptr;
    *fresh = false;
    uint32_t key[kConeKeyWords];
    const size_t bytes = cone_table_key(p, dz, shadow_nl, cls, lists, key);
    for (auto& t : im.tabs) {
        if (std::memcmp(t.key, key, sizeof key) != 0) continue;
        if (!t.done && t.stream != ctx->stream) {
            const hipError_t q = hipEventQuery(t.ready);
            if (q == hipSuccess) t.done = true;
            else if (q == hipErrorNotReady) RT_HIP(hipStreamWaitEvent(ctx->stream, t.ready, 0));
            else return hip_fail(q, "hipEventQuery");
        }
        *tab = &t;
        return RT_OK;
    }
    if (im.tabs.size() >= kMaxConeTabs) return RT_OK;
    if (im.tabs.capacity() < kMaxConeTabs) im.tabs.reserve(kMaxConeTabs);
    im.tabs.emplace_back();
    auto& t = im.tabs.back();
    std::memcpy(t.key, key, sizeof key);
    t.stream = ctx->stream;
    hipError_t e = t.buf.ensure(bytes);
    if (e == hipSuccess) e = hipEventCreateWithFlags(&t.ready, hipEventDisableTiming);
    if (e == hipSuccess && lists) {
        e = hipHostMalloc(reinterpret_cast<void**>(&t.counts), sizeof(unsigned long long));
        if (e == hipSuccess) __atomic_store_n(t.counts, 0ull, __ATOMIC_RELAXED);
    }
    if (e != hipSuccess) {
        t.buf.release();
        if (t.ready) (void)hipEventDestroy(t.ready);
        im.tabs.pop_back();
        return hip_fail(e, "cone table entry");
    }
    *tab = &t;
    *fresh = true;
    return RT_OK;
}

void cone_table_drop(rt_scene::PkImage& im) {
    auto& t = im.tabs.back();
    t.buf.release();
    if (t.ready) (void)hipEventDestroy(t.ready);
    if (t.counts) (void)hipHostFree(t.counts);
    im.tabs.pop_back();
}

rt_status cone_table_single(rt_context* ctx, const rt_scene* sc, rt_scene::PkImage& im,
                            TraceParams& p) {
    const TabsWanted want = tables_wanted(sc, p);
    if (!want.any()) return RT_OK;
    rt_scene::PkImage::ConeTab* t = nullptr;
    bool fresh = false;
    const rt_status st = cone_table_entry(ctx, im, p, p.cam_dz, want.shadow_nl, want.cls_kind(),
                                          false, &t, &fresh);
    if (st != RT_OK || !t) return st;
    if (fresh) {
        PkConeJobs jobs;
        std::memset(&jobs, 0, sizeof jobs);
        jobs.dst[0] = static_cast<unsigned long long*>(t->buf.ptr);
        jobs.frame[0] = -1;
        jobs.n = 1;
        jobs.shadow_nl = want.shadow_nl;
        jobs.class_words = want.cls_kind();
        hipError_t e = launch_packet_cone_tables(p, jobs, ctx->stream);
        if (e == hipSuccess) e = hipEventRecord(t->ready, ctx->stream);
        if (e != hipSuccess) {
            cone_table_drop(im);
            return hip_fail(e, "cone table setup");
        }
    }
    uint32_t key[kConeKeyWords];
    size_t tiles = 0;
    (void)cone_table_key(p, p.cam_dz, want.shadow_nl, want.cls_kind(), false, key, &tiles);
    const unsigned long long* words = static_cast<const unsigned long long*>(t->buf.ptr);
    if (want.cone) p.cone_tab = words;
    if (want.shadow) p.shadow_tab = words + tiles;
    if (want.cls) p.class_tab = words + tiles * (1 + static_cast<size_t>(want.shadow_nl));
    p.plane_masks = want.clear ? 1u : 0u;
    return RT_OK;
}

}

rt_status packet_image(rt_context* ctx, const rt_scene* sc, TraceParams& p, int flags,
                       rt_scene::PkImage::TileOrder** rec) {
    *rec = nullptr;
    rt_scene::PkImage* found = nullptr;
    rt_status st = packet_image_cached(ctx, sc, p.cam_pos, &found);
    if (st != RT_OK) return st;
    if (found) {
        p.pk_image = static_cast<const double*>(found->buf.ptr);
        st = tile_order(ctx, *found, p, flags, rec);
        return st != RT_OK ? st : cone_table_single(ctx, sc, *found, p);
    }
    if (!packet_second_sighting(sc, p.cam_pos)) {
        const rt_status st2 = packet_publish_slot(ctx, sc, p);
        return st2 != RT_OK ? st2 : scene_tile_order(ctx, sc, p, flags, rec);
    }
    rt_scene::PkImage* im = nullptr;
    st = packet_image_entry(ctx, sc, p.cam_pos, p, &im);
    if (st != RT_OK) return st;
    hipError_t e = launch_packet_image(p, static_cast<double*>(im->buf.ptr), ctx->stream);
    if (e == hipSuccess) e = hipEventRecord(im->ready, ctx->stream);
    if (e != hipSuccess) {
        im->buf.release();
        (void)hipEventDestroy(im->ready);
        sc->pk_images.pop_back();
        return hip_fail(e, "packet image setup");
    }
    p.pk_image = static_cast<const double*>(im->buf.ptr);
    st = tile_order(ctx, *im, p, flags, rec);
    return st != RT_OK ? st : cone_table_single(ctx, sc, *im, p);
}

rt_status packet_batch_images(rt_context* ctx, const rt_scene* sc, const rt_camera* cams,
                              int nframes, TraceParams& p, int flags,
                              rt_scene::PkImage::TileOrder** rec, int* batch_ring,
                              PkSplit* split) {
    *rec = nullptr;
    *batch_ring = -1;
    *split = PkSplit{0u, 0u, 0u};
    enum Kind { kCached, kPromote, kRing, kDup };
    Kind kind[kPkMaxBatch];
    int dup_of[kPkMaxBatch];
    rt_scene::PkImage* ent[kPkMaxBatch] = {};
    bool same_cam = true;
    bool any_ring = false;
    const size_t cache_before = sc->pk_images.size();
    struct Rollback {
        const rt_scene* sc;
        size_t keep;
        bool armed = true;
        ~Rollback() {
            if (!armed) return;
            while (sc->pk_images.size() > keep) {
                auto& im = sc->pk_images.back();
                im.buf.release();
                if (im.ready) (void)hipEventDestroy(im.ready);
                sc->pk_images.pop_back();
            }
        }
    } rollback{sc, cache_before};
    for (int f = 0; f < nframes; ++f) {
        PkFrame& F = p.fr[f];
        for (int i = 0; i < 3; ++i) F.cam[i] = cams[f].position[i];
        const CameraConsts cc = camera_consts(p.width, p.height, F.cam[2], p.focal);
        p.fr_dz[f][0] = cc.dz;
        p.fr_dz[f][1] = cc.dz2;
        F.img = nullptr;
        F.pub = nullptr;
        F.epoch = 0;
        F._pad = 0;
        if (std::memcmp(F.cam, p.fr[0].cam, sizeof F.cam) != 0) same_cam = false;
        int g = 0;
        while (g < f && std::memcmp(p.fr[g].cam, F.cam, sizeof F.cam) != 0) ++g;
        if (g < f) {
            kind[f] = kDup;
            dup_of[f] = g;
            continue;
        }
        rt_status st = packet_image_cached(ctx, sc, F.cam, &ent[f]);
        if (st != RT_OK) return st;
        if (ent[f]) {
            kind[f] = kCached;
            F.img = static_cast<const double*>(ent[f]->buf.ptr);
            continue;
        }
        if (packet_second_sighting(sc, F.cam)) {
            st = packet_image_entry(ctx, sc, F.cam, p, &ent[f]);
            if (st != RT_OK) return st;
            kind[f] = kPromote;
            F.img = static_cast<const double*>(ent[f]->buf.ptr);
            continue;
        }
        kind[f] = kRing;
        any_ring = true;
    }
    const size_t img_doubles = ((packet_lds_bytes(p.ns, p.np, p.nl) + 255) & ~size_t(255)) /
                               sizeof(double);
    double* ring = nullptr;
    if (any_ring) {
        const size_t entry = img_doubles * sizeof(double) * kPkMaxBatch;
        RT_HIP(sc->pk_batch.ensure(entry * rt_scene::kPkBatchRing));
        const int r = sc->pk_batch_next;
        sc->pk_batch_next = (r + 1) % rt_scene::kPkBatchRing;
        if (!sc->pk_batch_done[r])
            RT_HIP(hipEventCreateWithFlags(&sc->pk_batch_done[r], hipEventDisableTiming));
        if (sc->pk_batch_used[r])
            RT_HIP(hipStreamWaitEvent(ctx->stream, sc->pk_batch_done[r], 0));
        ring = reinterpret_cast<double*>(static_cast<char*>(sc->pk_batch.ptr) +
                                         static_cast<size_t>(r) * entry);
        *batch_ring = r;
    }
    PkImageJobs jobs;
    std::memset(&jobs, 0, sizeof jobs);
    for (int f = 0; f < nframes; ++f) {
        PkFrame& F = p.fr[f];
        if (kind[f] == kRing) F.img = ring + static_cast<size_t>(f) * img_doubles;
        if (kind[f] == kDup) F.img = p.fr[dup_of[f]].img;
        if (kind[f] == kRing || kind[f] == kPromote) {
            jobs.dst[jobs.n] = const_cast<double*>(F.img);
            jobs.frame[jobs.n] = f;
            ++jobs.n;
        }
    }
    hipError_t e = launch_packet_image_batch(p, jobs, ctx->stream);
    for (int f = 0; f < nframes && e == hipSuccess; ++f)
        if (kind[f] == kPromote) e = hipEventRecord(ent[f]->ready, ctx->stream);
    if (e != hipSuccess) return hip_fail(e, "packet batch images");
    rollback.armed = false;
    const rt_status ost = kind[0] == kCached ? tile_order(ctx, *ent[0], p, flags, rec, !same_cam)
                                             : scene_tile_order(ctx, sc, p, flags, rec);
    TabsWanted want = tables_wanted(sc, p);
    if (ost != RT_OK || !want.any()) return ost;
    if (any_ring) want.lists = false;
    uint32_t key[kConeKeyWords];
    size_t tiles = 0;
    const size_t tab_bytes =
        (cone_table_key(p, 0.0, want.shadow_nl, want.cls_kind(), want.lists, key, &tiles) + 255) &
        ~size_t(255);
    const size_t cone_bytes =
        (sizeof(unsigned long long) * tiles * (want.cls ? 2 : 1) + 255) & ~size_t(255);
    char* ring_tab = nullptr;
    size_t ring_room = 0;
    if (any_ring) {
        size_t n_ring = 0;
        for (int f = 0; f < nframes; ++f) n_ring += kind[f] == kRing;
        const size_t fit = std::min(n_ring, kConeRingBytes / cone_bytes);
        auto& buf = sc->pk_batch_tab[*batch_ring];
        if (fit > 0 && buf.bytes < fit * tab_bytes) {
            if (sc->pk_batch_used[*batch_ring])
                RT_HIP(hipEventSynchronize(sc->pk_batch_done[*batch_ring]));
            RT_HIP(buf.ensure(fit * tab_bytes));
        }
        ring_tab = static_cast<char*>(buf.ptr);
        ring_room = fit;
    }
    PkConeJobs cj;
    std::memset(&cj, 0, sizeof cj);
    cj.shadow_nl = want.shadow_nl;
    cj.class_words = want.cls_kind();
    cj.lists = want.lists ? 1 : 0;
    PkListCounts lc;
    std::memset(&lc, 0, sizeof lc);
    uint32_t gx, gy, waves;
    packet_grid(p, gx, gy, waves);
    uint32_t n_uni = 0, n_gen = 0;
    bool all_lists = want.lists;
    auto count_frame = [&](const unsigned long long* host) {
        const unsigned long long v = host ? __atomic_load_n(host, __ATOMIC_RELAXED) : 0ull;
        const uint32_t u = static_cast<uint32_t>(v), g = static_cast<uint32_t>(v >> 32);
        if (!u || !g) all_lists = false;
        n_uni = std::max(n_uni, u ? u - 1u : static_cast<uint32_t>(tiles));
        n_gen = std::max(n_gen, g ? g - 1u : gx * gy);
    };
    p.plane_masks = want.clear ? 1u : 0u;
    auto hand = [&](int f, const unsigned long long* words) {
        p.fr_tab[f] = want.cone ? words : nullptr;
        p.fr_stab[f] = want.shadow ? words + tiles : nullptr;
        p.fr_ctab[f] =
            want.cls ? words + tiles * (1 + static_cast<size_t>(want.shadow_nl)) : nullptr;
    };
    rt_scene::PkImage* made[kPkMaxBatch];
    rt_scene::PkImage::ConeTab* made_tab[kPkMaxBatch];
    int n_made = 0;
    rt_status st = RT_OK;
    for (int f = 0; f < nframes && st == RT_OK; ++f) {
        p.fr_tab[f] = nullptr;
        p.fr_stab[f] = nullptr;
        p.fr_ctab[f] = nullptr;
        unsigned long long* dst = nullptr;
        if (kind[f] == kDup) {
            p.fr_tab[f] = p.fr_tab[dup_of[f]];
            p.fr_stab[f] = p.fr_stab[dup_of[f]];
            p.fr_ctab[f] = p.fr_ctab[dup_of[f]];
            continue;
        }
        if (kind[f] == kRing) {
            if (ring_room == 0) all_lists = false;
            if (ring_room == 0) continue;
            --ring_room;
            dst = reinterpret_cast<unsigned long long*>(ring_tab);
            ring_tab += tab_bytes;
        } else {
            rt_scene::PkImage::ConeTab* t = nullptr;
            bool fresh = false;
            st = cone_table_entry(ctx, *ent[f], p, p.fr_dz[f][0], want.shadow_nl,
                                  want.cls_kind(), want.lists, &t, &fresh);
            if (st != RT_OK || !t) all_lists = false;
            if (st != RT_OK || !t) continue;
            hand(f, static_cast<const unsigned long long*>(t->buf.ptr));
            if (!fresh) count_frame(t->counts);
            if (!fresh) continue;
            lc.host[cj.n] = t->counts;
            made[n_made] = ent[f];
            made_tab[n_made] = t;
            ++n_made;
            dst = static_cast<unsigned long long*>(t->buf.ptr);
        }
        hand(f, dst);
        count_frame(nullptr);
        cj.dst[cj.n] = dst;
        cj.frame[cj.n] = f;
        ++cj.n;
    }
    if (st == RT_OK) {
        hipError_t ce = launch_packet_cone_tables(p, cj, ctx->stream, &lc);
        for (int i = 0; i < n_made && ce == hipSuccess; ++i)
            ce = hipEventRecord(made_tab[i]->ready, ctx->stream);
        if (ce != hipSuccess) st = hip_fail(ce, "packet batch cone tables");
    }
    if (st != RT_OK)
        for (int i = n_made - 1; i >= 0; --i) cone_table_drop(*made[i]);
    if (st == RT_OK && all_lists) {
        *split = PkSplit{static_cast<uint32_t>(tiles), n_uni, n_gen};
    }
    return st;
}

}
```

### raytracingengine_amd/csrc/rt_packet_kernel.hpp

```cpp
#pragma once

#include "rt_packet_device.hpp"
#include "rt_shadow_table.hpp"

#pragma clang fp contract(off)

namespace rtamd {

template <int MAXC, int FEAT>
__device__ __forceinline__ double pk_transmittance(const PacketScene& S, const Masks<MAXC>& M,
                                                   int nchunks, d3 o, d3 d, double max_dist,
                                                   double bias) {
    double T = 1.0, traveled = 0.0;
    int safety = 64;
    while (safety-- > 0 && T > 1e-4 && traveled < max_dist) {
        PkHit h;
        if (!closest_masked<MAXC, FEAT>(S, M, nchunks, o, d, h)) break;
        const double t = h.t;
        if (t <= 0.0) {
            o = o + d * bias;
            traveled += bias;
            continue;
        }
        if (t <= bias) {
// ... 97 lines not shown
    B.ok = false;
    if (!casting) return B;
    const bool bad = casting_lane && !(isfinite(so.x) && isfinite(so.y) && isfinite(so.z));
    B.c = lane_d3(so, __builtin_ctzll(casting));
    float r_lane = 0.0f;
    if (casting_lane) {
        const float dx = static_cast<float>(so.x - B.c.x), dy = static_cast<float>(so.y - B.c.y),
                    dz = static_cast<float>(so.z - B.c.z);
        r_lane = sqrt_f32(dot3f(dx, dy, dz, dx, dy, dz)) * (1.0f + 1e-5f);
    }
    B.R = wave_red<1>(r_lane);
    B.ok = !__ballot(bad) && isfinite(B.R);
    return B;
}

template <int MAXC, int FEAT>
__device__ __forceinline__ Masks<MAXC> shadow_masks(const PacketScene& S, bool casting_lane, d3 so,
                                                    d3 lcenter, double lrad, double bias) {
    const OriginBall B = origin_ball(casting_lane, so);
    return B.ok ? cull_capsule<MAXC, FEAT>(S, B.c, B.R, lcenter, lrad, bias)
                : all_candidates<MAXC>(S.ns);
}

template <int MAXC, int FEAT, bool COUNT, bool TAB = false>
__device__ __forceinline__ void pk_light(const PacketScene& S, bool active, d3 P, d3 n, d3 view,
                                         const PkHit& h, d3 lpos, d3 E, d3 lcenter, double lrad,
                                         double bias, int nchunks, d3& diff, d3& spec,
                                         Counts& cnt, const Masks<MAXC>* pre = nullptr,
                                         bool* fix = nullptr,
                                         const unsigned long long* stab = nullptr) {
    double dist = 0.0, inv_d2 = 0.0;
    d3 L = mk(0.0, 0.0, 0.0);
    if (active) light_dir(lpos - P, dist, L, inv_d2);
    const bool reach = active && !(dist <= 0.0);
    if (!reach) L = mk(0.0, 0.0, 0.0);
    const double ndl = smax(0.0, dot(n, L));
    const bool need = reach && !(ndl <= 0.0) && !(dist <= bias);
    const d3 so = P + n * bias;
    const uint64_t casting = __ballot(need);
    if (!casting) return;
    int occ = 0;
    Masks<MAXC> M;
    bool tabled = false;
    if constexpr (TAB) {
        if (stab) {
            const unsigned long long w = *(pk_culp)stab;
            if (w != ~0ull) {
                M.m[0] = w;
                M.pm = ~0ull;
                tabled = true;
            }
        }
    }
    if (pre) {
        M = *pre;
        if (need) occ = pk_occlusion<MAXC, FEAT>(S, M, nchunks, so, L, dist - bias, bias);
    } else if (TAB && tabled) {
        if (need) occ = pk_occlusion<MAXC, FEAT>(S, M, nchunks, so, L, dist - bias, bias);
    } else {
        const OriginBall B = origin_ball(need, so);
        M = B.ok ? cull_capsule<MAXC, FEAT>(S, B.c, B.R, lcenter, lrad, bias)
                 : all_candidates<MAXC>(S.ns);
        bool split = false;
        if constexpr (kShadowSplit && MAXC > 1) {
            int cand = 0;
#pragma unroll
            for (int c = 0; c < MAXC; ++c) cand += __builtin_popcountll(M.m[c]);
            split = B.ok && cand > kShadowSplitMin;
            if (split) {
                float r_lane = 0.0f;
                if (need) {
                    const float dx = static_cast<float>(so.x - B.c.x),
                                dy = static_cast<float>(so.y - B.c.y),
                                dz = static_cast<float>(so.z - B.c.z);
                    r_lane = sqrt_f32(dot3f(dx, dy, dz, dx, dy, dz));
                }
                const bool near = r_lane <= 0.5f * B.R;
                Masks<MAXC> Mn = M, Mf = M;
                const OriginBall Bn = origin_ball(need && near, so);
                const OriginBall Bf = origin_ball(need && !near, so);
                if (Bn.ok) {
                    const Masks<MAXC> t =
                        cull_capsule<MAXC, (FEAT & ~kFeatPlanes)>(S, Bn.c, Bn.R, lcenter, lrad, bias);
#pragma unroll
                    for (int c = 0; c < MAXC; ++c) Mn.m[c] &= t.m[c];
                    Mn.pm &= t.pm;
                }
                if (Bf.ok) {
                    const Masks<MAXC> t =
                        cull_capsule<MAXC, (FEAT & ~kFeatPlanes)>(S, Bf.c, Bf.R, lcenter, lrad, bias);
#pragma unroll
                    for (int c = 0; c < MAXC; ++c) Mf.m[c] &= t.m[c];
                    Mf.pm &= t.pm;
                }
#pragma unroll 1
                for (int g = 0; g < 2; ++g) {
                    Masks<MAXC> Mg;
#pragma unroll
                    for (int c = 0; c < MAXC; ++c) Mg.m[c] = g == 0 ? Mn.m[c] : Mf.m[c];
                    Mg.pm = g == 0 ? Mn.pm : Mf.pm;
                    if (need && near == (g == 0))
                        occ = pk_occlusion<MAXC, FEAT>(S, Mg, nchunks, so, L, dist - bias, bias);
                }
            }
        }
        if (!split && need) occ = pk_occlusion<MAXC, FEAT>(S, M, nchunks, so, L, dist - bias, bias);
    }
    const bool undecided = need && occ == 2;
    double T = occ == 1 ? 0.0 : 1.0;
    if constexpr ((FEAT & kFeatFix) != 0) {
        if (undecided) *fix = true;
    } else if (__ballot(undecided)) {
        Masks<MAXC> Mu = M;
        const OriginBall Bu = origin_ball(undecided, so);
        if (Bu.ok) {
            const Masks<MAXC> t = cull_capsule<MAXC, FEAT>(S, Bu.c, Bu.R, lcenter, lrad, bias);
#pragma unroll
            for (int c = 0; c < MAXC; ++c) Mu.m[c] &= t.m[c];
            Mu.pm &= t.pm;
        }
        if (undecided) T = pk_transmittance<MAXC, FEAT>(S, Mu, nchunks, so, L, dist - bias, bias);
    }
    if (!need) return;
    if (COUNT) cnt.shadow++;
    if (T <= bias) return;
    diff = diff + ((E * inv_d2) * ndl) * T;
    if constexpr ((FEAT & kFeatSpec) != 0) {
        const double* m = pk_material<MAXC>(S, h);
        if (m[5] <= 0.0 && m[4] > 0.0) {
            const d3 H = unit(L + view);
            const double ndh = smax(0.0, dot(n, H));
            if (ndh > 0.0) {
                const double sf = pow_bp(ndh, m[3]);
                spec = spec + ((E * inv_d2) * sf) * T;
            }
        }
    }
}

template <int MAXC>
__device__ __forceinline__ void pk_light_record(const PacketScene& S, const TraceParams& P, int l,
                                                d3& L, d3& E) {
    if constexpr (MAXC == 1) {
        const pk_cdp q = (pk_cdp)P.lt + kLtStride * l;
        L = mk(q[0], q[1], q[2]);
        E = mk(q[3], q[4], q[5]);
    } else {
        const double* q = S.lt + kLtStride * l;
        L = mk(q[0], q[1], q[2]);
        E = mk(q[3], q[4], q[5]);
    }
}

template <int MAXC, int FEAT>
__device__ __forceinline__ d3 pk_uniform_tile(const PacketScene& S, const TraceParams& P,
                                              const double* img, unsigned long long cls, d3 cam,
                                              d3 d, int ns, int np, int nl, double bias,
                                              bool& fix) {
    if (tile_class_of(cls) == kTileSky) return sky(d);
    const int k = static_cast<int>(tile_class_of(cls) - kTilePlane0);
    const pk_cdp pl = (pk_cdp)img + kPkSph * ns;
    const pk_cdp rec = pl + kPlStride * k;
    const pk_cdp on = pl + kPlStride * np + kLtStride * nl + 4 * k;
    const pk_cdp m = (pk_cdp)P.sph_mat + kMatStride * (ns + k);
    const pk_cdp oth = pl + kPlStride * (np > 1 ? 1 - k : k);
    const d3 pp = mk(rec[0], rec[1], rec[2]), pn = mk(rec[3], rec[4], rec[5]);
    const double num = rec[6], core = rec[7];
    const d3 n = mk(on[0], on[1], on[2]);
    bool found = false;
    double t = 0.0;
    int prim = -1;
    const double denom = dot(pn, d);
    if (core != 0.0) plane_t_core(num, denom, ns + k, found, t, prim);
    else plane_t(num, denom, ns + k, found, t, prim);
    const d3 hp = cam + d * t;
    d3 diff = mk(0.0, 0.0, 0.0);
    const d3 spec = mk(0.0, 0.0, 0.0);
    for (int l = 0; l < nl; ++l) {
        d3 lpos, E;
        pk_light_record<MAXC>(S, P, l, lpos, E);
        double dist = 0.0, inv_d2 = 0.0;
        d3 L = mk(0.0, 0.0, 0.0);
        light_dir(lpos - hp, dist, L, inv_d2);
        const bool reach = !(dist <= 0.0);
        if (!reach) L = mk(0.0, 0.0, 0.0);
        const double ndl = smax(0.0, dot(n, L));
        const bool need = reach && !(ndl <= 0.0) && !(dist <= bias);
        const d3 so = hp + n * bias;
        if (!__ballot(need)) continue;
        bool blocked = false, undecided = false;
        const unsigned keep = tile_plane_keep(cls, l);
        if (keep != 0 && need) {
            const double max_dist = dist - bias;
#pragma unroll
            for (int i = 0; i < 2; ++i) {
                if (i >= np) break;
                if (((keep >> (i == 0 ? k : 1 - k)) & 1u) == 0) continue;
                const d3 qp = i == 0 ? pp : mk(oth[0], oth[1], oth[2]);
                const d3 qn = i == 0 ? pn : mk(oth[3], oth[4], oth[5]);
                const double dn = dot(qn, L);
                if (!(fabs(dn) > 1e-6)) continue;
                const double nm = dot(qp - so, qn);
                const double A = dn > 0.0 ? nm : -nm, B = fabs(dn);
                if (A < -1e-300 * B) continue;
                if (A >= max_dist * B * (1.0 + 1e-9)) continue;
                if (A > bias * B * (1.0 + 1e-9) && A < max_dist * B * (1.0 - 1e-9)) blocked = true;
                else undecided = true;
            }
        }
        const double T = (!undecided && blocked) ? 0.0 : 1.0;
        if (undecided) fix = true;
        if (!need) continue;
        if (T <= bias) continue;
        diff = diff + ((E * inv_d2) * ndl) * T;
    }
    const d3 local = hmul(mk(m[0], m[1], m[2]), diff) + spec * m[4];
    const double tr = sclamp(m[5], 0.0, 1.0);
    d3 fin = mk(0.0, 0.0, 0.0);
    if (tr < 1.0) fin = fin + local * (1.0 - tr);
    return fin;
}

constexpr int pk_waves(int MAXC, int FEAT, bool COUNT, bool MULTI) {
    return (FEAT == (kFeatFix | kFeatSplit) && MAXC == 1 && !MULTI && !COUNT)
               ? RT_PACKET_GENERAL_WAVES
         : (FEAT == kFeatFix && MAXC == 1 && !MULTI && !COUNT) ? RT_PACKET_FIX_WAVES
         : (FEAT == 0 && MAXC == 1 && !MULTI && !COUNT) ? RT_PACKET_SMALL_WAVES
         : (FEAT == (kFeatArea | kFeatNoPL) && !MULTI && !COUNT) ? RT_PACKET_AREA_WAVES
         : FEAT == kFeatTris ? RT_PACKET_TRIS_WAVES
         : (((FEAT == 0 || (FEAT & ~kFeatNoPL) == kFeatArea || FEAT == kFeatPlanes) && MAXC <= 4)
                ? (MULTI ? (FEAT == 0 ? RT_PACKET_LEAN_WAVES : 1) : RT_PACKET_AA1_WAVES)
                : 1);
}
template <int MAXC, int FEAT_, bool COUNT, bool MULTI, int WGY>
__global__ __launch_bounds__(64 * kWgWavesX * WGY, pk_waves(MAXC, FEAT_, COUNT, MULTI)) void packet_direct_kernel(TraceParams P) {
    constexpr int FEAT = FEAT_ & ~kFeatSplit;
    constexpr bool SPLIT = (FEAT_ & kFeatSplit) != 0;
    extern __shared__ __attribute__((aligned(16))) double smem[];
    const int tid = threadIdx.x;
    constexpr bool kNoPL = (FEAT & kFeatNoPL) != 0;
    const uint32_t lin = blockIdx.y * gridDim.x + blockIdx.x;
    uint32_t tbx = blockIdx.x, tby = gridDim.y - 1 - blockIdx.y;
    const uint32_t gxw = SPLIT ? (P.width + kPkW * kWgWavesX - 1) / (kPkW * kWgWavesX) : gridDim.x;
    if constexpr (!SPLIT) {
        if (P.tile_order) {
            const uint32_t t = P.tile_order[lin];
            tbx = t % gridDim.x;
            tby = t / gridDim.x;
        }
    }
    uint64_t t_start = 0;
    if constexpr (MULTI)
        if (P.tile_cost) t_start = __builtin_amdgcn_s_memrealtime();
    const int ns = P.ns, np = kNoPL ? 0 : P.np, nl = kNoPL ? 0 : P.nl, nb = pk_chunk_bounds(ns),
              nsb = ns + nb;
    double* s_sph = smem;
    double* s_pl = s_sph + kPkSph * nsb;
    double* s_lt = s_pl + kPlStride * np;
    double* s_pln = s_lt + kLtStride * nl;
    const int32_t* s_orig = reinterpret_cast<const int32_t*>(s_pln + 4 * np);
    const double* camp = P.cam_pos;
    const double* pk_img = P.pk_image;
    unsigned long long* pk_pub = P.pk_pub;
    uint32_t pk_epoch = P.pk_epoch;
    uint64_t frame_off = 0;
    constexpr bool kLean = MAXC == 1 && (FEAT & kFeatArea) == 0;
    constexpr bool kTab = kLean && !MULTI && !COUNT && (FEAT == 0 || FEAT == kFeatFix);
    const unsigned long long* cone_tab = kTab ? P.cone_tab : nullptr;
    const unsigned long long* shadow_tab = kTab ? P.shadow_tab : nullptr;
    constexpr bool kUni = kTab && FEAT == kFeatFix && !SPLIT;
    const unsigned long long* class_tab = (kUni || SPLIT) ? P.class_tab : nullptr;
    double cam_dz = P.cam_dz, cam_dz2 = P.cam_dz2;
    if (P.nframes) {
        const PkFrame& F = P.fr[blockIdx.z];
        camp = F.cam;
        cam_dz = P.fr_dz[blockIdx.z][0];
        cam_dz2 = P.fr_dz[blockIdx.z][1];
        pk_img = F.img;
        pk_pub = F.pub;
        pk_epoch = F.epoch;
        frame_off = static_cast<uint64_t>(blockIdx.z) * P.frame_px;
        if constexpr (kTab) {
            cone_tab = P.fr_tab[blockIdx.z];
            shadow_tab = P.fr_stab[blockIdx.z];
        }
        if constexpr (kUni || SPLIT) class_tab = P.fr_ctab[blockIdx.z];
    }
    if constexpr (SPLIT) {
        const uint32_t split_tiles =
            gxw * ((P.rows + kPkH * WGY - 1) / (kPkH * WGY)) * (kWgWavesX * WGY);
        const pk_culp hdr = (pk_culp)class_tab + split_tiles;
        if (lin >= static_cast<uint32_t>(hdr[0] >> 32)) return;
        const uint32_t t = ((pk_cip)(hdr + 1 + split_tiles))[lin];
        tbx = t % gxw;
        tby = t / gxw;
    }
    const d3 cam = mk(camp[0], camp[1], camp[2]);
    constexpr int kThreads = 64 * kWgWavesX * WGY;
    unsigned long long cls = kTileGeneral;
    bool staged = true;
    if constexpr (kUni) {
        if (class_tab && pk_img && P.max_rec > 0) {
            const pk_culp cw =
                (pk_culp)class_tab + (tby * gxw + tbx) * (kWgWavesX * WGY);
            const uint32_t w = __builtin_amdgcn_readfirstlane(static_cast<uint32_t>(tid >> 6));
            bool all = true;
#pragma unroll
            for (uint32_t i = 0; i < kWgWavesX * WGY; ++i) {
                const unsigned long long c = cw[i];
                all = all && tile_class_of(c) != kTileGeneral;
                if (i == w) cls = c;
            }
            staged = !all;
        }
    }
    if constexpr (SPLIT) {
        const uint32_t w = __builtin_amdgcn_readfirstlane(static_cast<uint32_t>(tid >> 6));
        cls = ((pk_culp)class_tab)[(tby * gxw + tbx) * (kWgWavesX * WGY) + w];
    }
    if (pk_img && staged) {
        const float4* src = reinterpret_cast<const float4*>(pk_img);
        float4* dst = reinterpret_cast<float4*>(smem);
        const int nv = static_cast<int>(pk_image_bytes(ns, np, nl) / 16);
        for (int i = tid; i < nv; i += kThreads) dst[i] = src[i];
        __syncthreads();
        if constexpr (SPLIT)
            if (tile_class_of(cls) != kTileGeneral) return;
    } else if (pk_img) {
    } else if (pk_pub) {
        uint32_t* dst = reinterpret_cast<uint32_t*>(smem);
        const int nw = static_cast<int>(pk_image_bytes(ns, np, nl) / 4);
        const uint32_t ep = pk_epoch;
        const uint32_t wg = lin;
        bool have = false;
        if (wg >= P.pk_pub_first) {
            int ok = 1;
            for (int i = tid; i < nw / 2; i += kThreads) {
                const unsigned long long gx = __hip_atomic_load(
                    pk_pub + 2 * i, __ATOMIC_RELAXED, __HIP_MEMORY_SCOPE_AGENT);
                const unsigned long long gy = __hip_atomic_load(
                    pk_pub + 2 * i + 1, __ATOMIC_RELAXED, __HIP_MEMORY_SCOPE_AGENT);
                ok &= static_cast<uint32_t>(gx >> 32) == ep && static_cast<uint32_t>(gy >> 32) == ep;
                dst[2 * i] = static_cast<uint32_t>(gx);
                dst[2 * i + 1] = static_cast<uint32_t>(gy);
            }
            have = __syncthreads_and(ok) != 0;
        }
        if (!have) {
            pk_build_image(P, camp, smem, tid, kThreads);
            __syncthreads();
            if (wg == 0) {
                const unsigned long long tag = static_cast<unsigned long long>(ep) << 32;
                for (int i = tid; i < nw; i += kThreads)
                    __hip_atomic_store(pk_pub + i, tag | dst[i], __ATOMIC_RELAXED,
                                       __HIP_MEMORY_SCOPE_AGENT);
            }
        }
    } else {
        pk_build_image(P, camp, smem, tid, kThreads);
        __syncthreads();
    }

    PacketScene S;
    S.sph = s_sph;
    S.pl = s_pl;
    S.lt = s_lt;
    S.tri = P.tri;
    S.mat = P.sph_mat;
    S.bvh = P.bvh;
    S.bvh_tri = P.bvh_tri;
    S.ns = ns;
    S.np = np;
    S.nt = P.nt;
    S.nl = nl;
    S.nb = nb;
    S.orig = nb ? s_orig : nullptr;
    S.wstk = nullptr;
    if constexpr ((FEAT & kFeatTris) != 0)
        S.wstk = reinterpret_cast<int*>(smem + pk_image_bytes(ns, np, nl) / 8) +
                 kPkStack * (tid >> 6);
    const int nchunks = (ns + 63) / 64;

    const int lane = tid & 63, wave = tid >> 6;
    const uint32_t x = tbx * (kPkW * kWgWavesX) + (wave % kWgWavesX) * kPkW + (lane % kPkW);
    const uint32_t yl = tby * (kPkH * WGY) + (wave / kWgWavesX) * kPkH + (lane / kPkW);
    const bool valid = x < P.width && yl < P.rows;
    const uint32_t xc = x < P.width ? x : P.width - 1;
    const uint32_t y = image_row(P, yl < P.rows ? yl : P.rows - 1);
    const uint64_t pix = static_cast<uint64_t>(y) * P.width + xc;
    const double bias = P.bias;
    d3 al_c = mk(0.0, 0.0, 0.0);
    double al_r = 0.0;
    if constexpr ((FEAT & kFeatArea) != 0) {
        const d3 eu = mk(P.al_u[0], P.al_u[1], P.al_u[2]);
        const d3 ev = mk(P.al_v[0], P.al_v[1], P.al_v[2]);
        al_c = (mk(P.al_corner[0], P.al_corner[1], P.al_corner[2]) + eu * 0.5) + ev * 0.5;
        al_r = (0.5 * (length(eu) + length(ev))) * (1.0 + kCullRel);
    }
    Counts cnt{0u, 0u};
    bool fix = false;

    d3 acc = mk(0.0, 0.0, 0.0);
    int samples = 0;
    const int nsamples = MULTI ? P.aa : 1;
    for (int s = 0; s < nsamples; ++s) {
        d3 d;
        if constexpr (kLean) {
            double sx = static_cast<double>(xc) - P.half_w;
            double sy = P.half_h - static_cast<double>(y);
            if constexpr (MULTI) {
                double jx = 0.0, jy = 0.0;
                if (s > 0 && P.aa > 1) {
                    jx = u01(P.seed, pix, static_cast<uint32_t>(s), 0u);
                    jy = u01(P.seed, pix, static_cast<uint32_t>(s), 1u);
                }
                sx += jx;
                sy += jy;
            }
            const d3 dv = mk(sx - cam.x, sy - cam.y, cam_dz);
            d = unit_sq(dv, dv.x * dv.x + dv.y * dv.y + cam_dz2);
        } else {
            d = camera_dir(P, cam, xc, y, pix, s);
        }

        d3 col;
        if (P.max_rec <= 0) {
            col = sky(d);
        } else if (kUni && tile_class_of(cls) != kTileGeneral) {
            if constexpr (kUni)
                col = pk_uniform_tile<MAXC, FEAT>(S, P, pk_img, cls, cam, d, ns, np, nl, bias, fix);
        } else {
            if (COUNT && valid) cnt.trace++;
            const Masks<MAXC> M = [&] {
                if constexpr (kTab) {
                    if (cone_tab) {
                        Masks<MAXC> T;
                        const uint32_t w =
                            __builtin_amdgcn_readfirstlane(static_cast<uint32_t>(wave));
                        T.m[0] = ((pk_culp)cone_tab)[(tby * gxw + tbx) * (kWgWavesX * WGY) + w];
                        T.pm = ~0ull;
                        return T;
                    }
                }
                const d3 axis = lane_d3(d, (kPkH / 2) * kPkW + kPkW / 2);
                const double cos_min =
                    static_cast<double>(wave_red<0>(static_cast<float>(dot(d, axis)))) - 1e-7;
                const bool ok = isfinite(cos_min) && cos_min > 0.0;
                return ok ? cull_cone<MAXC>(S, axis, cos_min) : all_candidates<MAXC>(ns);
            }();
            PkHit h;
            h.t = 0.0;
            h.prim = 0;
            const bool hit = valid && closest_camera<MAXC, FEAT>(S, M, nchunks, cam, d, h);
            const d3 hp = cam + d * h.t;
            d3 view = mk(0.0, 0.0, 0.0);
            d3 inc = mk(0.0, 0.0, 0.0);
            if constexpr ((FEAT & kFeatSpec) != 0) {
                inc = unit(d);
                view = -inc;
            }
            d3 n = mk(0.0, 1.0, 0.0);
            bool known = !hit;
            if (hit && h.prim >= ns && h.prim < ns + np) {
                const double* q = s_pln + 4 * (h.prim - ns);
                if (q[3] != 0.0) {
                    n = mk(q[0], q[1], q[2]);
                    known = true;
                }
            }
            if (!known) {
                const d3 gn = pk_normal(S, h, hp);
                bool front;
                if constexpr ((FEAT & kFeatSpec) != 0) {
                    front = dot(gn, inc) < 0.0;
                } else {
                    const double nd = dot(gn, d);
                    const double sabs = fabs(gn.x * d.x) + fabs(gn.y * d.y) + fabs(gn.z * d.z);
                    if (fabs(nd) > 1e-14 * sabs && sabs > 1e-200) front = nd < 0.0;
                    else front = dot(gn, unit(d)) < 0.0;
                }
// ... 130 lines not shown
```

### raytracingengine_amd/csrc/rt_shadow_table.hpp

```cpp
#pragma once

#include <math.h>
#include <stddef.h>
#include <stdint.h>

#include "rt_cone_table.hpp"

#if defined(__clang__)
#define RT_ST_UNROLL _Pragma("unroll")
#else
#define RT_ST_UNROLL
#endif

namespace rtamd {

constexpr int kShadowTabLights = 4;
constexpr int kShadowTabPlanes = 8;
constexpr unsigned long long kShadowNoWord = ~0ull;
constexpr double kClassMargin = 1e-6;
constexpr unsigned long long kTileGeneral = 0ull, kTileSky = 1ull, kTilePlane0 = 2ull;

RT_CT_HD inline int shadow_table_lights(int ns, int np, int nl, bool area_light) {
    return (!area_light && ns >= 1 && ns <= 63 && np >= 1 && np <= kShadowTabPlanes && nl >= 1 &&
            nl <= kShadowTabLights)
// ... 56 lines not shown
            const double mag = (fabs(a) + fabs(b)) + fabs(c);
            if (!isfinite(ek) || !(fabs(ek) <= 0x1p200)) return B;
            if (ek > 1e-12 * mag) ++n_hit;
            else if (ek <= 0.0) ++n_miss;
            if (fabs(ek) < e_min) e_min = fabs(ek);
            e[i][k] = ek;
        }
        if (n_miss == 4) {
            hit[i] = false;
        } else if (n_hit == 4 && e_min * e_min >= 4e-12 * vl2_max) {
            hit[i] = true;
        } else {
            return B;
        }
    }
    RT_ST_UNROLL
    for (int j = 0; j < kMaxPlanes; ++j) {
        if (j >= np) break;
        if (!hit[j]) continue;
        bool hidden = false;
    RT_ST_UNROLL
        for (int i = 0; i < kMaxPlanes; ++i) {
            if (i >= np || hidden) break;
            if (i == j || !hit[i]) continue;
            int ahead = 0;
            for (int k = 0; k < kHideCorners; ++k) {
                const double lhs = e[i][k] * an[j], rhs = e[j][k] * an[i];
                ahead += lhs >= rhs * (1.0 + 1e-9) && rhs >= 0x1p-900;
            }
            hidden = ahead == kHideCorners;
        }
        if (hidden) continue;
        ShadowBall& S = B.ball[B.n];
        S.plane = j;
        S.lead = true;
    RT_ST_UNROLL
        for (int i = 0; i < kMaxPlanes; ++i) {
            if (i >= np) break;
            if (i == j || !hit[i]) continue;
            int ahead = 0;
            for (int k = 0; k < kHideCorners; ++k) {
                const double lhs = e[j][k] * an[i], rhs = e[i][k] * an[j];
                ahead += lhs >= rhs * (1.0 + kClassMargin) && rhs >= 0x1p-900;
            }
            S.lead = S.lead && ahead == kHideCorners;
        }
        double h[4][3];
        S.c[0] = S.c[1] = S.c[2] = 0.0;
        const double e01 = e[j][0] * e[j][1], e23 = e[j][2] * e[j][3];
        const double scale = an[j] / (e01 * e23);
        if (!(e01 * e23 >= 0x1p-900) || !isfinite(scale)) return B;
        const double tk[4] = {scale * (e[j][1] * e23), scale * (e[j][0] * e23),
                              scale * (e01 * e[j][3]), scale * (e01 * e[j][2])};
        for (int k = 0; k < kCorners; ++k) {
            const double t = tk[k];
            for (int a = 0; a < 3; ++a) {
                h[k][a] = cam[a] + v[k][a] * t;
                S.c[a] += h[k][a] / kCorners;
            }
        }
        double r2 = 0.0;
        for (int k = 0; k < kCorners; ++k) {
            const double dx = h[k][0] - S.c[0], dy = h[k][1] - S.c[1], dz_ = h[k][2] - S.c[2];
            const double d2 = dx * dx + dy * dy + dz_ * dz_;
            if (d2 > r2) r2 = d2;
        }
        const double R = static_cast<double>(sqrtf(static_cast<float>(r2) * (1.0f + 1e-6f)) *
                                             (1.0f + 1e-6f));
        const double c1 = fabs(S.c[0]) + fabs(S.c[1]) + fabs(S.c[2]);
        const double Rm = R + 1e-8 * ((cam1 + c1) + R);
        if (!isfinite(Rm) || !isfinite(c1)) return B;
        S.R = static_cast<float>(Rm) * (1.0f + 1e-5f);
        if (kBiasInR) S.R += static_cast<float>(fabs(bias)) * (1.0f + 1e-6f) * 1.001f;
        if (!isfinite(S.R)) return B;
        ++B.n;
    }
    B.ok = true;
    return B;
}

struct ShadowSeg {
    float sx, sy, sz, sl2, inv_sl2, Rc;
    bool huge;
};
RT_CT_HD inline ShadowSeg shadow_seg(const double* c, float R, const double* L, double bias) {
    ShadowSeg G;
    G.sx = static_cast<float>(L[0] - c[0]);
    G.sy = static_cast<float>(L[1] - c[1]);
    G.sz = static_cast<float>(L[2] - c[2]);
    G.sl2 = G.sx * G.sx + G.sy * G.sy + G.sz * G.sz;
    G.inv_sl2 = 1.0f / G.sl2;
    G.huge = !(G.sl2 <= 0x1p120f);
    G.Rc = (R > 0.0f ? R : 0.0f) + static_cast<float>(fabs(bias)) * (1.0f + 1e-6f) * 1.001f;
    return G;
}
RT_CT_HD inline bool shadow_seg_keeps(const ShadowSeg& G, const double* c, const double* s,
                                      float r) {
    const float vx = static_cast<float>(s[0] - c[0]), vy = static_cast<float>(s[1] - c[1]),
                vz = static_cast<float>(s[2] - c[2]);
    const float vs = vx * G.sx + vy * G.sy + vz * G.sz;
    const float vv = vx * vx + vy * vy + vz * vz;
    float d2;
    if (!(vs > 0.0f) || !(G.sl2 > 0.0f)) {
        d2 = vv;
    } else if (!(vs < G.sl2)) {
        const float wx = vx - G.sx, wy = vy - G.sy, wz = vz - G.sz;
        d2 = wx * wx + wy * wy + wz * wz;
    } else {
        d2 = vv - (vs * vs) * G.inv_sl2;
    }
    const float lim = (r + G.Rc) * (1.0f + 1e-4f);
    const float far = 1e5f * r - G.Rc;
    return !(d2 > lim * lim + 2e-5f * (vv + G.sl2)) || !(far > 0.0f) || !(vv <= far * far) ||
           G.huge;
}
RT_CT_HD inline bool shadow_keeps(const double* c, float R, const double* L, double bias,
                                  const double* s, float r) {
    return shadow_seg_keeps(shadow_seg(c, R, L, bias), c, s, r);
}

template <int kMaxPlanes>
RT_CT_HD inline unsigned long long shadow_tile_word(const ShadowBound<kMaxPlanes>& B,
                                                    const double* L, double bias,
                                                    const double* sph, int sph_stride,
                                                    const float* rad, int rad_stride, int ns) {
    if (!B.ok || ns > 63) return kShadowNoWord;
    unsigned long long m = 0;
    RT_ST_UNROLL
    for (int b = 0; b < kMaxPlanes; ++b) {
        if (b >= B.n) break;
        const ShadowSeg G = shadow_seg(B.ball[b].c, B.ball[b].R, L, bias);
        for (int i = 0; i < ns; ++i)
            if (shadow_seg_keeps(G, B.ball[b].c, sph + static_cast<long>(sph_stride) * i,
                                 rad[static_cast<long>(rad_stride) * i]))
                m |= 1ull << i;
    }
    return m;
}

template <int kMaxPlanes, int kClassPlanes = 1, int kIndexOff = 0>
RT_CT_HD inline unsigned long long tile_class_word(unsigned long long cone,
                                                   const ShadowBound<kMaxPlanes>& B,
                                                   const unsigned long long* words, int nl,
                                                   const double* pln, int np) {
    if (cone != 0 || !B.ok || B.n > kClassPlanes || nl < 1 || nl > kShadowTabLights)
        return kTileGeneral;
    for (int l = 0; l < nl; ++l)
        if (words[l] != 0) return kTileGeneral;
    if (B.n == 0) return kTileSky;
    const int i = B.ball[0].plane;
    if (kClassPlanes == 1 && !B.ball[0].lead) return kTileGeneral;
    if (i < 0 || i >= np || !(pln[4 * i + 3] != 0.0)) return kTileGeneral;
    return kTilePlane0 + static_cast<unsigned long long>((i + kIndexOff) % np);
}

constexpr unsigned kPlaneKeepAll = 0xffu;
template <int kMaxPlanes, bool kSideOfBall = true>
RT_CT_HD inline unsigned shadow_plane_keep(const ShadowBound<kMaxPlanes>& B, const double* L,
                                           const double* planes, int np, const double* cam,
                                           double bias) {
    if (!B.ok || np < 1 || np > kMaxPlanes || np > 8) return kPlaneKeepAll;
    const double ab = fabs(bias);
    const double base = ((fabs(cam[0]) + fabs(cam[1])) + fabs(cam[2])) +
                        ((fabs(L[0]) + fabs(L[1])) + fabs(L[2])) + ab;
    unsigned keep = 0;
    RT_ST_UNROLL
    for (int i = 0; i < kMaxPlanes; ++i) {
        if (i >= np) break;
        const double* p = planes + 8 * i;
        const double N = sqrt((p[3] * p[3] + p[4] * p[4]) + p[5] * p[5]);
        const double p1 = (fabs(p[0]) + fabs(p[1])) + fabs(p[2]);
        const double sL = ((L[0] - p[0]) * p[3] + (L[1] - p[1]) * p[4]) + (L[2] - p[2]) * p[5];
        bool drop = N >= 0x1p-21 && N <= 2.0;
        RT_ST_UNROLL
        for (int b = 0; b < kMaxPlanes; ++b) {
            if (b >= B.n) break;
            const ShadowBall& S = B.ball[b];
            const double R = static_cast<double>(S.R);
            const double scale =
                (base + p1) + (((fabs(S.c[0]) + fabs(S.c[1])) + fabs(S.c[2])) + R);
            if (!(scale >= 0x1p-200 && scale <= 0x1p200)) drop = false;
            if (S.plane == i) {
                if (!(bias >= 1e-7 * scale)) drop = false;
                continue;
            }
            const double m = 1e-6 * scale * N;
            const double sc =
                ((S.c[0] - p[0]) * p[3] + (S.c[1] - p[1]) * p[4]) + (S.c[2] - p[2]) * p[5];
            if (!((sL > 0.0 && sc > 0.0) || (sL < 0.0 && sc < 0.0)) && kSideOfBall) drop = false;
            if (!(fabs(sc) - R * N >= m) && kSideOfBall) drop = false;
            if (!(fabs(sL) - 2.0 * ab * N >= m)) drop = false;
        }
        if (!drop) keep |= 1u << i;
    }
    return keep;
}

constexpr unsigned long long kTileClassBits = 0xffull;
RT_CT_HD inline unsigned long long tile_class_of(unsigned long long word) {
    return word & kTileClassBits;
}
RT_CT_HD inline unsigned long long tile_class_pack(unsigned long long cls, const unsigned* keep,
                                                   int nl) {
    unsigned long long w = cls & kTileClassBits;
    for (int l = 0; l < nl && l < kShadowTabLights; ++l)
        w |= static_cast<unsigned long long>(keep[l] & kPlaneKeepAll) << (8 + 8 * l);
    return w;
}
RT_CT_HD inline unsigned tile_plane_keep(unsigned long long word, int l) {
    return static_cast<unsigned>(word >> (8 + 8 * l)) & kPlaneKeepAll;
}

constexpr int kListColShift = 40, kListRowShift = 52;
constexpr unsigned long long kListWordMask = (1ull << kListColShift) - 1ull;
constexpr uint32_t kListCoordMask = 0xfffu;
constexpr uint32_t kListMaxCoord = kListCoordMask + 1u;
RT_CT_HD inline size_t tile_list_words(size_t tiles, size_t wgs) {
    return 1 + tiles + (wgs + 1) / 2;
}
RT_CT_HD inline uint32_t tile_list_tile(uint32_t pos, uint32_t tiles) { return tiles - 1u - pos; }
RT_CT_HD inline bool tile_list_uniform(unsigned long long word) {
    return tile_class_of(word) != kTileGeneral;
}
template <int kIndexOff = 0>
RT_CT_HD inline unsigned long long tile_list_entry(unsigned long long word, uint32_t x0,
                                                   uint32_t yl0) {
    return (word & kListWordMask) |
           (static_cast<unsigned long long>((x0 / 8u + kIndexOff) & kListCoordMask) << kListColShift) |
           (static_cast<unsigned long long>((yl0 / 8u) & kListCoordMask) << kListRowShift);
}
template <bool kDropMixed = false>
RT_CT_HD inline bool tile_list_wg_listed(uint64_t general, unsigned lane, unsigned waves) {
    const uint64_t group = (waves >= 64u ? ~0ull : (1ull << waves) - 1ull);
    const uint64_t g = (general >> (lane & ~(waves - 1u))) & group;
    return kDropMixed ? g == group : g != 0;
}
template <int kIndexOff = 0, bool kDropMixed = false, class Origin>
inline void tile_list_run(const unsigned long long* words, uint32_t tiles, uint32_t waves,
                          uint32_t pos0, Origin origin, unsigned long long* uni, uint32_t* n_uni,
                          uint32_t* gen, uint32_t* n_gen) {
    uint64_t general = 0;
    for (uint32_t l = 0; l < 64 && pos0 + l < tiles; ++l)
        if (!tile_list_uniform(words[tile_list_tile(pos0 + l, tiles)])) general |= 1ull << l;
    for (uint32_t l = 0; l < 64 && pos0 + l < tiles; ++l) {
        const uint32_t t = tile_list_tile(pos0 + l, tiles);
        if (tile_list_uniform(words[t])) {
            uint32_t x0, yl0;
            origin(t, x0, yl0);
            uni[(*n_uni)++] = tile_list_entry<kIndexOff>(words[t], x0, yl0);
        }
        if ((l & (waves - 1u)) == 0 && tile_list_wg_listed<kDropMixed>(general, l, waves))
            gen[(*n_gen)++] = t / waves;
    }
}

}
```

Baseline: 159,300.

## Route single-plane tiles shadowed by spheres to the uniform tile kernel

Adds a third tile class: tiles whose primary hit is a single plane but whose shadow rays may hit spheres. These tiles get a marker bit, are listed in a separate shadowed list at the end of the uniform buffer, and are rendered by a templated uniform kernel that tests shadow rays against only the spheres named in the tile's shadow-table word. The general per-pixel kernel then skips them. The aim is to move such tiles off the expensive general path onto the cheaper uniform path, at the cost of an extra launch, more list bookkeeping, and an additional atomic counter.

```diff
diff --git a/include/rt_capi.h b/include/rt_capi.h
--- a/include/rt_capi.h
+++ b/include/rt_capi.h
@@ -373,6 +373,10 @@
 
 rt_status rt_debug_tile_split(rt_context* ctx, uint64_t* split, uint64_t* single);
 
+rt_status rt_debug_tile_shadowed(rt_context* ctx, uint64_t* with, uint64_t* without);
+
+rt_status rt_debug_fixup_count(rt_context* ctx, uint32_t* pixels);
+
 #ifdef __cplusplus
 }
 #endif
diff --git a/raytracingengine_amd/capi.py b/raytracingengine_amd/capi.py
--- a/raytracingengine_amd/capi.py
+++ b/raytracingengine_amd/capi.py
@@ -78,6 +78,7 @@
     "rt_debug_tile_class",
     "rt_debug_plane_clear",
     "rt_debug_tile_split",
+    "rt_debug_tile_shadowed", "rt_debug_fixup_count",
     "rt_occluded_rays", "rt_occluded_rays_device",
     "rt_transmittance_rays", "rt_transmittance_rays_device",
     "rt_light_transmittance", "rt_light_transmittance_device",
@@ -274,6 +275,8 @@
         "rt_debug_tile_class": [vp, vp, vp],
         "rt_debug_plane_clear": [vp, vp, vp],
         "rt_debug_tile_split": [vp, vp, vp],
+        "rt_debug_tile_shadowed": [vp, vp, vp],
+        "rt_debug_fixup_count": [vp, vp],
         "rt_debug_assemble_rows": [vp, vp, ctypes.c_size_t, ctypes.c_uint32, ctypes.c_uint32,
                                    ctypes.c_uint32, ctypes.c_uint32, vp],
     }.items():
@@ -426,6 +429,16 @@
         a, b = ctypes.c_uint64(), ctypes.c_uint64()
         _check(_lib.rt_debug_tile_split(self._h, ctypes.byref(a), ctypes.byref(b)))
         return a.value, b.value
+
+    def debug_tile_shadowed(self) -> tuple[int, int]:
+        a, b = ctypes.c_uint64(), ctypes.c_uint64()
+        _check(_lib.rt_debug_tile_shadowed(self._h, ctypes.byref(a), ctypes.byref(b)))
+        return a.value, b.value
+
+    def debug_fixup_count(self) -> int:
+        n = ctypes.c_uint32()
+        _check(_lib.rt_debug_fixup_count(self._h, ctypes.byref(n)))
+        return n.value
 
     def debug_vec_ops(self, v: np.ndarray) -> np.ndarray:
         v = np.ascontiguousarray(v, np.float64).reshape(-1, 3)
diff --git a/raytracingengine_amd/csrc/rt_capi.cpp b/raytracingengine_amd/csrc/rt_capi.cpp
--- a/raytracingengine_amd/csrc/rt_capi.cpp
+++ b/raytracingengine_amd/csrc/rt_capi.cpp
@@ -347,6 +347,9 @@
     if (!fixup || p.tile_order) pk_split.tiles = 0;
     if (packet && fixup)
         (pk_split.tiles ? ctx->tile_split_frames : ctx->tile_nosplit_frames) += nframes;
+    if (packet && fixup)
+        ((pk_split.tiles && pk_split.sh_n) ? ctx->tile_shadowed_frames
+                                           : ctx->tile_noshadowed_frames) += nframes;
     const bool lean_generic = p.nt == 0 && p.al_samples == 0;
     static const bool box_sph = [] {
         const char* e = std::getenv("RTAMD_BOX_SPH");
@@ -1807,6 +1810,25 @@
     return RT_OK;
 }
 
+rt_status rt_debug_tile_shadowed(rt_context* ctx, uint64_t* with, uint64_t* without) {
+    if (!ctx || !with || !without)
+        return fail(RT_ERR_INVALID_ARG, "NULL argument to rt_debug_tile_shadowed");
+    *with = ctx->tile_shadowed_frames;
+    *without = ctx->tile_noshadowed_frames;
+    return RT_OK;
+}
+
+rt_status rt_debug_fixup_count(rt_context* ctx, uint32_t* pixels) {
+    if (!ctx || !pixels) return fail(RT_ERR_INVALID_ARG, "NULL argument to rt_debug_fixup_count");
+    *pixels = 0;
+    if (!ctx->fix_ctl.ptr) return RT_OK;
+    DeviceGuard g(ctx->device);
+    RT_HIP(hipStreamSynchronize(ctx->stream));
+    RT_HIP(hipMemcpy(pixels, static_cast<const uint32_t*>(ctx->fix_ctl.ptr) + (1 - ctx->fix_parity),
+                     sizeof(uint32_t), hipMemcpyDeviceToHost));
+    return RT_OK;
+}
+
 rt_status rt_debug_vec_ops(rt_context* ctx, const double* v, size_t n, double* out) {
     if (!ctx || !v || !out) return fail(RT_ERR_INVALID_ARG, "NULL argument");
     DeviceGuard g(ctx->device);
diff --git a/raytracingengine_amd/csrc/rt_context.hpp b/raytracingengine_amd/csrc/rt_context.hpp
--- a/raytracingengine_amd/csrc/rt_context.hpp
+++ b/raytracingengine_amd/csrc/rt_context.hpp
@@ -77,6 +77,7 @@
     uint64_t tile_class_frames = 0, tile_noclass_frames = 0;
     uint64_t plane_mask_frames = 0, plane_nomask_frames = 0;
     uint64_t tile_split_frames = 0, tile_nosplit_frames = 0;
+    uint64_t tile_shadowed_frames = 0, tile_noshadowed_frames = 0;
     std::vector<rt_context*> group_ctxs;
     std::vector<rt_comm*> group_comms;
     std::vector<rt_context*> group_roots;
diff --git a/raytracingengine_amd/csrc/rt_internal.hpp b/raytracingengine_amd/csrc/rt_internal.hpp
--- a/raytracingengine_amd/csrc/rt_internal.hpp
+++ b/raytracingengine_amd/csrc/rt_internal.hpp
@@ -101,6 +101,7 @@
 struct PkSplit {
     uint32_t tiles;
     uint32_t uni_n, gen_n;
+    uint32_t sh_n;
 };
 static_assert(sizeof(TraceParams) + 12 * kPkMaxBatch + 32 <= 4096, "kernel arguments above 4 KiB");
 
diff --git a/raytracingengine_amd/csrc/rt_packet.hip b/raytracingengine_amd/csrc/rt_packet.hip
--- a/raytracingengine_amd/csrc/rt_packet.hip
+++ b/raytracingengine_amd/csrc/rt_packet.hip
@@ -86,7 +86,9 @@
     }
     if (J.class_words == 0) return;
     const double* pln = img + kPkSph * ns + kPlStride * P.np + kLtStride * P.nl;
-    const unsigned long long cw = tile_class_word(cone, SB, &any, 1, pln, P.np) | keep;
+    const unsigned long long mark =
+        J.lists == 2 ? tile_shadowed_mark(cone, SB, &any, 1, pln, P.np) : 0ull;
+    const unsigned long long cw = tile_class_word(cone, SB, &any, 1, pln, P.np) | keep | mark;
     J.dst[blockIdx.y][static_cast<size_t>(gx) * gy * waves * (1 + J.shadow_nl) + t] = cw;
     if (!J.lists) return;
     const size_t tiles = static_cast<size_t>(gx) * gy * waves;
@@ -94,33 +96,47 @@
     unsigned long long* uni = hdr + 1;
     uint32_t* gen = reinterpret_cast<uint32_t*>(hdr + 1 + tiles);
     const uint32_t lane = threadIdx.x & 63u;
-    const bool is_uni = tile_list_uniform(cw);
-    const uint64_t bu = __ballot(is_uni), bg = __ballot(!is_uni);
+    const bool is_uni = tile_list_uniform(cw), is_sh = tile_list_shadowed(cw);
+    const uint64_t bu = __ballot(is_uni), bs = __ballot(is_sh), bg = __ballot(!is_uni && !is_sh);
     const bool lead = (lane & (waves - 1u)) == 0 && tile_list_wg_listed(bg, lane, waves);
     const uint64_t bl = __ballot(lead);
-    uint32_t base_u = 0, base_g = 0;
+    uint32_t base_u = 0, base_g = 0, base_s = 0;
     if (lane == 0) {
         if (bu) base_u = atomicAdd(reinterpret_cast<uint32_t*>(hdr),
                                    static_cast<uint32_t>(__builtin_popcountll(bu)));
         if (bl) base_g = atomicAdd(reinterpret_cast<uint32_t*>(hdr) + 1,
                                    static_cast<uint32_t>(__builtin_popcountll(bl)));
+        if (bs)
+            base_s = atomicAdd(reinterpret_cast<uint32_t*>(
+                                   hdr + tile_list_shadowed_count(tiles, static_cast<size_t>(gx) * gy)),
+                               static_cast<uint32_t>(__builtin_popcountll(bs)));
     }
     base_u = __shfl(base_u, 0, 64);
     base_g = __shfl(base_g, 0, 64);
+    base_s = __shfl(base_s, 0, 64);
     const uint64_t below = (1ull << lane) - 1ull;
     if (is_uni) uni[base_u + __builtin_popcountll(bu & below)] = tile_list_entry(cw, x0, yl0);
+    if (is_sh)
+        uni[tile_list_shadowed_slot(base_s + __builtin_popcountll(bs & below),
+                                    static_cast<uint32_t>(tiles))] = tile_shadowed_entry(cw, x0, yl0);
     if (lead) gen[base_g + __builtin_popcountll(bl & below)] = wg;
 }
 
-__global__ __launch_bounds__(64) void packet_list_zero_kernel(PkConeJobs J, size_t hdr) {
-    if (static_cast<int>(threadIdx.x) < J.n) J.dst[threadIdx.x][hdr] = 0ull;
+__global__ __launch_bounds__(64) void packet_list_zero_kernel(PkConeJobs J, size_t hdr,
+                                                              size_t hdr_s) {
+    if (static_cast<int>(threadIdx.x) >= J.n) return;
+    J.dst[threadIdx.x][hdr] = 0ull;
+    J.dst[threadIdx.x][hdr_s] = 0ull;
 }
 __global__ __launch_bounds__(64) void packet_list_counts_kernel(PkConeJobs J, PkListCounts C,
-                                                                size_t hdr) {
+                                                                size_t hdr, size_t hdr_s) {
     if (static_cast<int>(threadIdx.x) >= J.n || !C.host[threadIdx.x]) return;
     const unsigned long long v = J.dst[threadIdx.x][hdr];
+    const unsigned long long s = J.dst[threadIdx.x][hdr_s];
     __hip_atomic_store(C.host[threadIdx.x],
                        (((v >> 32) + 1ull) << 32) | ((v & 0xffffffffull) + 1ull), __ATOMIC_RELAXED,
+                       __HIP_MEMORY_SCOPE_SYSTEM);
+    __hip_atomic_store(C.host[threadIdx.x] + 1, (s & 0xffffffffull) + 1ull, __ATOMIC_RELAXED,
                        __HIP_MEMORY_SCOPE_SYSTEM);
 }
 
@@ -134,6 +150,7 @@
     if (jobs.class_words != 0 && jobs.shadow_nl <= 0) return hipErrorInvalidValue;
     if (jobs.class_words < 0 || jobs.class_words > 2) return hipErrorInvalidValue;
     if (jobs.lists != 0 && jobs.class_words == 0) return hipErrorInvalidValue;
+    if (jobs.lists < 0 || jobs.lists > 2) return hipErrorInvalidValue;
     for (int j = 0; j < jobs.n; ++j) {
         const int f = jobs.frame[j];
         if (!jobs.dst[j] || f < -1 || f >= static_cast<int>(p.nframes) ||
@@ -144,10 +161,12 @@
     packet_grid(p, gx, gy, waves);
     const uint32_t tiles = gx * gy * waves;
     const size_t hdr = static_cast<size_t>(tiles) * (2 + jobs.shadow_nl);
+    const size_t hdr_s = hdr + tile_list_shadowed_count(tiles, static_cast<size_t>(gx) * gy);
     if (jobs.lists) {
         if (gx * kWgWavesX > kListMaxCoord || gy * (waves / kWgWavesX) > kListMaxCoord)
             return hipErrorInvalidValue;
-        hipLaunchKernelGGL(packet_list_zero_kernel, dim3(1), dim3(64), 0, stream, jobs, hdr);
+        hipLaunchKernelGGL(packet_list_zero_kernel, dim3(1), dim3(64), 0, stream, jobs, hdr,
+                           hdr_s);
     }
     hipLaunchKernelGGL(packet_cone_table_kernel,
                        dim3((tiles + kConeThreads - 1) / kConeThreads,
@@ -155,7 +174,7 @@
                        dim3(kConeThreads), 0, stream, p, jobs, gx, gy, waves);
     if (jobs.lists && counts)
         hipLaunchKernelGGL(packet_list_counts_kernel, dim3(1), dim3(64), 0, stream, jobs, *counts,
-                           hdr);
+                           hdr, hdr_s);
     return hipGetLastError();
 }
 
@@ -337,14 +356,16 @@
 #define RT_PACKET_UNI_WAVES 8
 #endif
 constexpr int kUniThreads = RT_PACKET_UNI_THREADS;
+template <bool SPH>
 __global__ __launch_bounds__(kUniThreads, RT_PACKET_UNI_WAVES) void packet_uniform_kernel(TraceParams P, uint32_t tiles) {
     constexpr int FEAT = kFeatFix;
     const PkFrame& F = P.fr[blockIdx.z];
     const pk_culp hdr = (pk_culp)P.fr_ctab[blockIdx.z] + tiles;
     const uint32_t i = blockIdx.x * (kUniThreads / 64) +
                        __builtin_amdgcn_readfirstlane(static_cast<uint32_t>(threadIdx.x) >> 6);
-    if (i >= static_cast<uint32_t>(hdr[0])) return;
-    const unsigned long long e = hdr[1 + i];
+    if (i >= static_cast<uint32_t>(hdr[SPH ? tile_list_shadowed_count(tiles, tiles / kWgWavesX) : 0]))
+        return;
+    const unsigned long long e = hdr[1 + (SPH ? tile_list_shadowed_slot(i, tiles) : i)];
     const unsigned long long cls = e & kListWordMask;
     const uint32_t col = static_cast<uint32_t>(e >> kListColShift) & kListCoordMask;
     const uint32_t row = static_cast<uint32_t>(e >> kListRowShift) & kListCoordMask;
@@ -362,7 +383,16 @@
     bool fix = false;
     PacketScene S;
     S.lt = nullptr;
-    const d3 col3 = pk_uniform_tile<1, FEAT>(S, P, F.img, cls, cam, d, P.ns, P.np, P.nl, P.bias, fix);
+    d3 col3;
+    if constexpr (SPH) {
+        const uint32_t cols = (P.width + kPkW * kWgWavesX - 1) / (kPkW * kWgWavesX) * kWgWavesX;
+        const unsigned long long* stab =
+            P.fr_stab[blockIdx.z] + static_cast<size_t>(row * cols + col) * P.nl;
+        col3 = pk_uniform_tile<1, FEAT, true>(S, P, F.img, cls, cam, d, P.ns, P.np, P.nl, P.bias,
+                                              fix, stab);
+    } else {
+        col3 = pk_uniform_tile<1, FEAT>(S, P, F.img, cls, cam, d, P.ns, P.np, P.nl, P.bias, fix);
+    }
     const d3 acc = mk(0.0, 0.0, 0.0) + col3;
     constexpr int samples = 1;
     const uint32_t lane_e = lane, x_e = x, yl_e = yl;
@@ -383,13 +413,17 @@
     const dim3 block(64 * kWgWavesX);
     const dim3 ggrid(s.gen_n, 1u, p.nframes);
     const dim3 ugrid((s.uni_n + kUniThreads / 64 - 1) / (kUniThreads / 64), 1u, p.nframes);
+    const dim3 sgrid((s.sh_n + kUniThreads / 64 - 1) / (kUniThreads / 64), 1u, p.nframes);
 #ifdef RT_PACKET_SPLIT_GENERAL_FIRST
     if (s.gen_n)
         hipLaunchKernelGGL((packet_direct_kernel<1, kFeatFix | kFeatSplit, false, false, 1>),
                            ggrid, block, lds, stream, p);
 #endif
     if (s.uni_n)
-        hipLaunchKernelGGL(packet_uniform_kernel, ugrid, dim3(kUniThreads), 0, stream, p,
+        hipLaunchKernelGGL(packet_uniform_kernel<false>, ugrid, dim3(kUniThreads), 0, stream, p,
+                           s.tiles);
+    if (s.sh_n)
+        hipLaunchKernelGGL(packet_uniform_kernel<true>, sgrid, dim3(kUniThreads), 0, stream, p,
                            s.tiles);
 #ifndef RT_PACKET_SPLIT_GENERAL_FIRST
     if (s.gen_n)
diff --git a/raytracingengine_amd/csrc/rt_packet_host.cpp b/raytracingengine_amd/csrc/rt_packet_host.cpp
--- a/raytracingengine_amd/csrc/rt_packet_host.cpp
+++ b/raytracingengine_amd/csrc/rt_packet_host.cpp
@@ -173,11 +173,13 @@
     bool cls;
     bool clear;
     bool lists;
+    bool shadowed;
+    int list_kind() const { return lists ? (shadowed ? 2 : 1) : 0; }
     int cls_kind() const { return cls ? (clear ? 2 : 1) : 0; }
     bool any() const { return cone || shadow; }
 };
 TabsWanted tables_wanted(const rt_scene* sc, const TraceParams& p) {
-    TabsWanted w{false, false, 0, false, false, false};
+    TabsWanted w{false, false, 0, false, false, false, false};
     if (!packet_reads_cone_table(p, sc->max_specular > 0.0)) return w;
     const char* e = std::getenv("RTAMD_PK_CONE_TAB");
     w.cone = !(e && std::atoi(e) == 0);
@@ -190,11 +192,13 @@
     w.clear = w.cls && !(e && std::atoi(e) == 0);
     w.lists = w.cls && p.nframes >= 1 && packet_uses_fixup(p, false, sc->max_specular > 0.0) &&
               packet_split_wanted(p);
+    e = std::getenv("RTAMD_PK_TILE_SHADOWED");
+    w.shadowed = w.lists && !(e && std::atoi(e) == 0);
     return w;
 }
 
 constexpr size_t kConeKeyWords = rt_scene::PkImage::ConeTab::kKeyWords;
-size_t cone_table_key(const TraceParams& p, double dz, int shadow_nl, int cls, bool lists,
+size_t cone_table_key(const TraceParams& p, double dz, int shadow_nl, int cls, int lists,
                       uint32_t (&key)[kConeKeyWords], size_t* tiles = nullptr) {
     uint32_t gx, gy, waves;
     packet_grid(p, gx, gy, waves);
@@ -209,7 +213,8 @@
     if (shadow_nl > 0) {
         key[15] = static_cast<uint32_t>(shadow_nl);
         std::memcpy(key + 16, &p.bias, sizeof p.bias);
-        key[18] = (cls == 2 ? 3u : (cls ? 1u : 0u)) | (cls && lists ? 4u : 0u);
+        key[18] = (cls == 2 ? 3u : (cls ? 1u : 0u)) | (cls && lists ? 4u : 0u) |
+                  (cls && lists == 2 ? 8u : 0u);
     }
     const size_t n = static_cast<size_t>(gx) * gy * waves;
     if (tiles) *tiles = n;
@@ -219,7 +224,7 @@
 }
 
 rt_status cone_table_entry(rt_context* ctx, rt_scene::PkImage& im, const TraceParams& p,
-                           double dz, int shadow_nl, int cls, bool lists,
+                           double dz, int shadow_nl, int cls, int lists,
                            rt_scene::PkImage::ConeTab** tab, bool* fresh) {
     *tab = nullptr;
     *fresh = false;
@@ -245,8 +250,9 @@
     hipError_t e = t.buf.ensure(bytes);
     if (e == hipSuccess) e = hipEventCreateWithFlags(&t.ready, hipEventDisableTiming);
     if (e == hipSuccess && lists) {
-        e = hipHostMalloc(reinterpret_cast<void**>(&t.counts), sizeof(unsigned long long));
+        e = hipHostMalloc(reinterpret_cast<void**>(&t.counts), 2 * sizeof(unsigned long long));
         if (e == hipSuccess) __atomic_store_n(t.counts, 0ull, __ATOMIC_RELAXED);
+        if (e == hipSuccess) __atomic_store_n(t.counts + 1, 0ull, __ATOMIC_RELAXED);
     }
     if (e != hipSuccess) {
         t.buf.release();
@@ -274,7 +280,7 @@
     rt_scene::PkImage::ConeTab* t = nullptr;
     bool fresh = false;
     const rt_status st = cone_table_entry(ctx, im, p, p.cam_dz, want.shadow_nl, want.cls_kind(),
-                                          false, &t, &fresh);
+                                          0, &t, &fresh);
     if (st != RT_OK || !t) return st;
     if (fresh) {
         PkConeJobs jobs;
@@ -293,7 +299,7 @@
     }
     uint32_t key[kConeKeyWords];
     size_t tiles = 0;
-    (void)cone_table_key(p, p.cam_dz, want.shadow_nl, want.cls_kind(), false, key, &tiles);
+    (void)cone_table_key(p, p.cam_dz, want.shadow_nl, want.cls_kind(), 0, key, &tiles);
     const unsigned long long* words = static_cast<const unsigned long long*>(t->buf.ptr);
     if (want.cone) p.cone_tab = words;
     if (want.shadow) p.shadow_tab = words + tiles;
@@ -341,7 +347,7 @@
                               PkSplit* split) {
     *rec = nullptr;
     *batch_ring = -1;
-    *split = PkSplit{0u, 0u, 0u};
+    *split = PkSplit{0u, 0u, 0u, 0u};
     enum Kind { kCached, kPromote, kRing, kDup };
     Kind kind[kPkMaxBatch];
     int dup_of[kPkMaxBatch];
@@ -435,11 +441,11 @@
                                              : scene_tile_order(ctx, sc, p, flags, rec);
     TabsWanted want = tables_wanted(sc, p);
     if (ost != RT_OK || !want.any()) return ost;
-    if (any_ring) want.lists = false;
+    if (any_ring) want.lists = want.shadowed = false;
     uint32_t key[kConeKeyWords];
     size_t tiles = 0;
     const size_t tab_bytes =
-        (cone_table_key(p, 0.0, want.shadow_nl, want.cls_kind(), want.lists, key, &tiles) + 255) &
+        (cone_table_key(p, 0.0, want.shadow_nl, want.cls_kind(), want.list_kind(), key, &tiles) + 255) &
         ~size_t(255);
     const size_t cone_bytes =
         (sizeof(unsigned long long) * tiles * (want.cls ? 2 : 1) + 255) & ~size_t(255);
@@ -462,19 +468,22 @@
     std::memset(&cj, 0, sizeof cj);
     cj.shadow_nl = want.shadow_nl;
     cj.class_words = want.cls_kind();
-    cj.lists = want.lists ? 1 : 0;
+    cj.lists = want.list_kind();
     PkListCounts lc;
     std::memset(&lc, 0, sizeof lc);
     uint32_t gx, gy, waves;
     packet_grid(p, gx, gy, waves);
-    uint32_t n_uni = 0, n_gen = 0;
+    uint32_t n_uni = 0, n_gen = 0, n_sh = 0;
     bool all_lists = want.lists;
     auto count_frame = [&](const unsigned long long* host) {
         const unsigned long long v = host ? __atomic_load_n(host, __ATOMIC_RELAXED) : 0ull;
+        const unsigned long long v2 = host ? __atomic_load_n(host + 1, __ATOMIC_RELAXED) : 0ull;
         const uint32_t u = static_cast<uint32_t>(v), g = static_cast<uint32_t>(v >> 32);
-        if (!u || !g) all_lists = false;
+        const uint32_t s = static_cast<uint32_t>(v2);
+        if (!u || !g || !s) all_lists = false;
         n_uni = std::max(n_uni, u ? u - 1u : static_cast<uint32_t>(tiles));
         n_gen = std::max(n_gen, g ? g - 1u : gx * gy);
+        n_sh = std::max(n_sh, s ? s - 1u : static_cast<uint32_t>(tiles));
     };
     p.plane_masks = want.clear ? 1u : 0u;
     auto hand = [&](int f, const unsigned long long* words) {
@@ -508,7 +517,7 @@
             rt_scene::PkImage::ConeTab* t = nullptr;
             bool fresh = false;
             st = cone_table_entry(ctx, *ent[f], p, p.fr_dz[f][0], want.shadow_nl,
-                                  want.cls_kind(), want.lists, &t, &fresh);
+                                  want.cls_kind(), want.list_kind(), &t, &fresh);
             if (st != RT_OK || !t) all_lists = false;
             if (st != RT_OK || !t) continue;
             hand(f, static_cast<const unsigned long long*>(t->buf.ptr));
@@ -535,7 +544,7 @@
     if (st != RT_OK)
         for (int i = n_made - 1; i >= 0; --i) cone_table_drop(*made[i]);
     if (st == RT_OK && all_lists) {
-        *split = PkSplit{static_cast<uint32_t>(tiles), n_uni, n_gen};
+        *split = PkSplit{static_cast<uint32_t>(tiles), n_uni, n_gen, want.shadowed ? n_sh : 0u};
     }
     return st;
 }
diff --git a/raytracingengine_amd/csrc/rt_packet_kernel.hpp b/raytracingengine_amd/csrc/rt_packet_kernel.hpp
--- a/raytracingengine_amd/csrc/rt_packet_kernel.hpp
+++ b/raytracingengine_amd/csrc/rt_packet_kernel.hpp
@@ -273,11 +273,12 @@
     }
 }
 
-template <int MAXC, int FEAT>
+template <int MAXC, int FEAT, bool SPH = false>
 __device__ __forceinline__ d3 pk_uniform_tile(const PacketScene& S, const TraceParams& P,
                                               const double* img, unsigned long long cls, d3 cam,
                                               d3 d, int ns, int np, int nl, double bias,
-                                              bool& fix) {
+                                              bool& fix,
+                                              const unsigned long long* stab = nullptr) {
     if (tile_class_of(cls) == kTileSky) return sky(d);
     const int k = static_cast<int>(tile_class_of(cls) - kTilePlane0);
     const pk_cdp pl = (pk_cdp)img + kPkSph * ns;
@@ -311,7 +312,55 @@
         if (!__ballot(need)) continue;
         bool blocked = false, undecided = false;
         const unsigned keep = tile_plane_keep(cls, l);
-        if (keep != 0 && need) {
+        bool planes = true;
+        if constexpr (SPH) {
+            const unsigned long long w = *(pk_culp)(stab + l);
+            if (w != 0 && need) {
+                const double max_dist = dist - bias;
+                const double a = dot(L, L);
+                const double two_a = 2.0 * a, four_a = 4.0 * a;
+                if (!(two_a >= 0x1p-100 && two_a <= 0x1p100)) {
+                    undecided = true;
+                    planes = false;
+                } else {
+                    const double inv2a = rcp_refined(two_a);
+                    uint64_t m = w;
+                    while (m) {
+                        const int i = __builtin_ctzll(m);
+                        m &= m - 1;
+                        const pk_cdp s = (pk_cdp)img + kPkSph * i;
+                        const d3 oc = so - mk(s[0], s[1], s[2]);
+                        const double b = 2.0 * dot(oc, L);
+                        const double cc = dot(oc, oc) - s[3];
+                        const double disc = b * b - four_a * cc;
+                        if (disc < 0.0) continue;
+                        if (!(disc == 0.0 || (disc > 1e-30 && disc < 1e30))) {
+                            undecided = true;
+                            continue;
+                        }
+                        const double sq = static_cast<double>(sqrt_f32(static_cast<float>(disc)));
+                        const double delta = 2e-6 * (fabs(b) + sq) * inv2a;
+                        double ts = (-b - sq) * inv2a;
+                        if (!(ts >= 1e-6 + delta)) {
+                            if (!(ts < 1e-6 - delta)) {
+                                undecided = true;
+                                continue;
+                            }
+                            ts = (-b + sq) * inv2a;
+                            if (ts < 1e-6 - delta) continue;
+                            if (!(ts >= 1e-6 + delta)) {
+                                undecided = true;
+                                continue;
+                            }
+                        }
+                        if (ts >= max_dist + delta) continue;
+                        if (ts > bias + delta && ts < max_dist - delta) blocked = true;
+                        else undecided = true;
+                    }
+                }
+            }
+        }
+        if (keep != 0 && need && planes) {
             const double max_dist = dist - bias;
 #pragma unroll
             for (int i = 0; i < 2; ++i) {
@@ -446,7 +495,7 @@
         for (int i = tid; i < nv; i += kThreads) dst[i] = src[i];
         __syncthreads();
         if constexpr (SPLIT)
-            if (tile_class_of(cls) != kTileGeneral) return;
+            if (tile_class_of(cls) != kTileGeneral || (cls & kTileShadowedBit) != 0) return;
     } else if (pk_img) {
     } else if (pk_pub) {
         uint32_t* dst = reinterpret_cast<uint32_t*>(smem);
diff --git a/raytracingengine_amd/csrc/rt_shadow_table.hpp b/raytracingengine_amd/csrc/rt_shadow_table.hpp
--- a/raytracingengine_amd/csrc/rt_shadow_table.hpp
+++ b/raytracingengine_amd/csrc/rt_shadow_table.hpp
@@ -232,6 +232,27 @@
     if (kClassPlanes == 1 && !B.ball[0].lead) return kTileGeneral;
     if (i < 0 || i >= np || !(pln[4 * i + 3] != 0.0)) return kTileGeneral;
     return kTilePlane0 + static_cast<unsigned long long>((i + kIndexOff) % np);
+}
+
+constexpr unsigned long long kTileShadowedBit = 1ull << 40;
+constexpr int kTileShadowedPlaneShift = 41;
+template <int kMaxPlanes, bool kNoWordOk = false, int kIndexOff = 0>
+RT_CT_HD inline unsigned long long tile_shadowed_mark(unsigned long long cone,
+                                                      const ShadowBound<kMaxPlanes>& B,
+                                                      const unsigned long long* words, int nl,
+                                                      const double* pln, int np) {
+    if ((cone != 0 && !kNoWordOk) || !B.ok || B.n != 1 || nl < 1 || nl > kShadowTabLights)
+        return 0ull;
+    bool some = false;
+    for (int l = 0; l < nl; ++l) {
+        if (words[l] == kShadowNoWord && !kNoWordOk) return 0ull;
+        some = some || words[l] != 0;
+    }
+    if (!some || !B.ball[0].lead) return 0ull;
+    const int i = B.ball[0].plane;
+    if (i < 0 || i >= np || i >= 8 || !(pln[4 * i + 3] != 0.0)) return 0ull;
+    return kTileShadowedBit |
+           (static_cast<unsigned long long>((i + kIndexOff) % np) << kTileShadowedPlaneShift);
 }
 
 constexpr unsigned kPlaneKeepAll = 0xffu;
@@ -296,7 +317,13 @@
 constexpr uint32_t kListCoordMask = 0xfffu;
 constexpr uint32_t kListMaxCoord = kListCoordMask + 1u;
 RT_CT_HD inline size_t tile_list_words(size_t tiles, size_t wgs) {
+    return 2 + tiles + (wgs + 1) / 2;
+}
+RT_CT_HD inline size_t tile_list_shadowed_count(size_t tiles, size_t wgs) {
     return 1 + tiles + (wgs + 1) / 2;
+}
+RT_CT_HD inline uint32_t tile_list_shadowed_slot(uint32_t j, uint32_t tiles) {
+    return tiles - 1u - j;
 }
 RT_CT_HD inline uint32_t tile_list_tile(uint32_t pos, uint32_t tiles) { return tiles - 1u - pos; }
 RT_CT_HD inline bool tile_list_uniform(unsigned long long word) {
@@ -334,4 +361,35 @@
     }
 }
 
-}
+RT_CT_HD inline bool tile_list_shadowed(unsigned long long word) {
+    return tile_class_of(word) == kTileGeneral && (word & kTileShadowedBit) != 0;
+}
+RT_CT_HD inline unsigned long long tile_shadowed_entry(unsigned long long word, uint32_t x0,
+                                                       uint32_t yl0) {
+    const unsigned long long cls = kTilePlane0 + ((word >> kTileShadowedPlaneShift) & 7ull);
+    return tile_list_entry((word & ~kTileClassBits) | cls, x0, yl0);
+}
+template <bool kDropShadowedMixed = false, class Origin>
+inline void tile_list_run3(const unsigned long long* words, uint32_t tiles, uint32_t waves,
+                           uint32_t pos0, Origin origin, unsigned long long* uni, uint32_t* n_uni,
+                           uint32_t* n_sh, uint32_t* gen, uint32_t* n_gen) {
+    uint64_t general = 0, shadowed = 0;
+    for (uint32_t l = 0; l < 64 && pos0 + l < tiles; ++l) {
+        const unsigned long long w = words[tile_list_tile(pos0 + l, tiles)];
+        if (tile_list_shadowed(w)) shadowed |= 1ull << l;
+        else if (!tile_list_uniform(w)) general |= 1ull << l;
+    }
+    for (uint32_t l = 0; l < 64 && pos0 + l < tiles; ++l) {
+        const uint32_t t = tile_list_tile(pos0 + l, tiles);
+        uint32_t x0, yl0;
+        origin(t, x0, yl0);
+        if (tile_list_uniform(words[t])) uni[(*n_uni)++] = tile_list_entry(words[t], x0, yl0);
+        else if (tile_list_shadowed(words[t]))
+            uni[tile_list_shadowed_slot((*n_sh)++, tiles)] = tile_shadowed_entry(words[t], x0, yl0);
+        if ((l & (waves - 1u)) == 0 && tile_list_wg_listed(general, l, waves) &&
+            !(kDropShadowedMixed && tile_list_wg_listed(shadowed, l, waves)))
+            gen[(*n_gen)++] = t / waves;
+    }
+}
+
+}
```

New measurement: 167,000 (median of 6 runs). +4.9%, better.
